# patriciogonzalezvivo/prisma

Measured on AMD Instinct MI355X. Metric: frames/sec (depth_anything ViT-L + flow_raft, 1080p), higher is better.
Workload: dtype split-f16

## Files before the change

include/prisma_bands.h:

```cpp
#ifndef PRISMA_BANDS_H
#define PRISMA_BANDS_H

#include <stddef.h>
#include <stdint.h>

#ifdef __cplusplus
extern "C" {
#endif

typedef struct pb_ctx pb_ctx;

typedef enum {
    PB_OK = 0,
    PB_ERR_ARG = -1,
    PB_ERR_DEVICE = -2,
    PB_ERR_MEMORY = -3,
    PB_ERR_STATE = -4
} pb_status;

typedef enum { PB_F32 = 0, PB_F16 = 1, PB_U8 = 2, PB_I32 = 3 } pb_dtype;

typedef struct {
    const char *name;
    int32_t dtype;
// ... 102 lines not shown
                           float *flow_out, uint8_t *rgb_out, float *maxdisp_out);
int pb_flow_infer_sequence_dev(pb_ctx *ctx, const uint8_t *frames, int F, int H, int W, float scale, int iters, int backward,
                               float *flow_out, uint8_t *rgb_out, float *maxdisp_out);
int pb_flow_infer_sequence_masks(pb_ctx *ctx, const uint8_t *frames, int F, int H, int W, float scale, int iters,
                                 float alpha1, float alpha2, float *flow_out, uint8_t *rgb_out, float *maxdisp_out,
                                 uint8_t *mask_out);
int pb_flow_infer_sequence_masks_dev(pb_ctx *ctx, const uint8_t *frames, int F, int H, int W, float scale, int iters,
                                     float alpha1, float alpha2, float *flow_out, uint8_t *rgb_out, float *maxdisp_out,
                                     uint8_t *mask_out);
int pb_flow_fwdbwd_mask(pb_ctx *ctx, const float *flows, int n, int sh, int sw, float alpha1, float alpha2,
                        uint8_t *mask_out);
int pb_flow_num_scales(pb_ctx *ctx);
int64_t pb_flow_get_stage(pb_ctx *ctx, const char *name, float *out, int64_t cap, int64_t shape_out[4]);
int pb_flow_set_inference_size(pb_ctx *ctx, int h, int w);
int pb_flow_set_matching(pb_ctx *ctx, int corr_radius, int prop_radius);
int pb_flow_set_alternate_corr(pb_ctx *ctx, int on);
int64_t pb_flow_arena_bytes(pb_ctx *ctx);

int pb_mask_infer_batch(pb_ctx *ctx, const uint8_t *frames, int n, int H, int W, float confidence,
                        const int32_t *keep_classes, int n_keep, uint8_t *mask_out);
int pb_mask_infer_batch_dev(pb_ctx *ctx, const uint8_t *frames, int n, int H, int W, float confidence,
                            const int32_t *keep_classes, int n_keep, uint8_t *mask_out);
int pb_mask_get_instances(pb_ctx *ctx, int frame, int cap, float *scores_out, int32_t *labels_out, uint8_t *masks_out,
                          int32_t *candidates_out);
int pb_mask_net_size(const pb_mask_cfg *cfg, int H, int W, int *nh, int *nw, int *Hp, int *Wp);
int pb_mask_set_sdf(pb_ctx *ctx, const uint8_t *tab_out, const uint8_t *tab_in, int n_tab);
int pb_mask_sdf_green(pb_ctx *ctx, uint8_t *masks, int n, int H, int W);
int pb_mask_sdf_green_dev(pb_ctx *ctx, uint8_t *masks, int n, int H, int W);
int64_t pb_mask_get_stage(pb_ctx *ctx, const char *name, float *out, int64_t cap, int64_t shape_out[4]);

int64_t pb_depth_get_stage(pb_ctx *ctx, const char *name, float *out, int64_t cap, int64_t shape_out[4]);

int pb_dev_alloc(pb_ctx *ctx, void **ptr, size_t bytes);
int pb_dev_free(pb_ctx *ctx, void *ptr);
int pb_memcpy_h2d(pb_ctx *ctx, void *dst, const void *src, size_t bytes);
int pb_memcpy_d2h(pb_ctx *ctx, void *dst, const void *src, size_t bytes);

typedef struct {
    const char *name;
    double ms;
    double flops;
    double exec_flops;
    double bytes;
    int32_t launches;
} pb_kernel_stat;
int pb_set_profiling(pb_ctx *ctx, int enabled);
int pb_set_option(pb_ctx *ctx, const char *key, int value);
int pb_get_kernel_stats(pb_ctx *ctx, pb_kernel_stat *out, int cap);

int pb_op_gemm(pb_ctx *ctx, const float *A, const float *W, const float *bias, float *C,
               int M, int N, int K, int act , int tile );
int pb_op_gemm_bench(pb_ctx *ctx, int M, int N, int K, int tile, int epi, int iters, double *ms_out);
int pb_op_corr_volume(pb_ctx *ctx, const float *A, int M, const float *W, int N, int ldo, int guard_rows, float *out);
int pb_op_attention_bench(pb_ctx *ctx, int B, int heads, int N, int variant, int iters, double *ms_out);
int pb_op_layernorm(pb_ctx *ctx, const float *x, const float *g, const float *b, float *y, int rows, int D);
int pb_op_attention(pb_ctx *ctx, const float *q, const float *k, const float *v, float *o,
                    int B, int heads, int N);
int pb_op_attention128(pb_ctx *ctx, const float *q, const float *k, const float *v, const int8_t *region, float *o, int B, int L);
int pb_op_attention128_split(pb_ctx *ctx, const float *q, const float *k, const float *v, const int8_t *region, int nreg, float *o,
                             int B, int L, int vcols, int kxor);
int pb_op_conv2d(pb_ctx *ctx, const float *x, const float *w, const float *bias, float *y,
                 int B, int Ci, int H, int W, int Co, int ksize, int stride, int pad, int relu_in, int relu_out);
int pb_op_conv2d_split(pb_ctx *ctx, const float *x, const float *w, const float *bias, const float *skip, int B, int H, int W, int Ci, int Ctot,
                       int ci_off, int Co, int kh, int kw, int stride, int layout, int sa, int tapin, int tile, int split_out, int act,
                       int pre_relu, int rows_out, void *out, int *info, char *kernel, int kernel_cap);
int pb_op_dense_split(pb_ctx *ctx, const float *A, const float *w, const float *bias, const float *skip, int M, int K, int N, int layout,
                      int sa, int tile, int split_out, int act, int rows_out, void *out, int *info, char *kernel, int kernel_cap);
int pb_op_gemm_resid(pb_ctx *ctx, const float *A, const float *w, const float *bias, const float *gamma, const float *X, int M, int N, int K, int ldr,
                     int layout, int tile, int guard_rows, float *out, int *info, char *kernel, int kernel_cap);
int pb_op_gemm_qkv(pb_ctx *ctx, const float *A, const float *w, const float *bias, int B, int ntp, int D, int layout, int tile, int guard_rows, void *q,
                   void *k, void *vt, int *info, char *kernel, int kernel_cap);
int pb_op_gemm_patch(pb_ctx *ctx, const float *A, const float *w, const float *bias, const float *pos, int B, int P, int ntp, int D, int layout,
                     int guard_rows, float *out, int *info, char *kernel, int kernel_cap);
int pb_op_raft_gru_zr(pb_ctx *ctx, const float *x, const float *w, const float *bias, const float *add1, const float *add2, float *h32, int n, int H, int W,
                      int gc, int kh, int kw, int layout, int tile, int guard_rows, void *zrb, void *rh, int *info, char *kernel, int kernel_cap);
int pb_op_raft_gru_q(pb_ctx *ctx, const float *x, const float *w, const float *bias, const float *add1, const float *add2, const float *z, float *h32, int n,
                     int H, int W, int gc, int kh, int kw, int layout, int tile, int guard_rows, void *out, int *info, char *kernel, int kernel_cap);
int pb_op_conv_pixshuf(pb_ctx *ctx, const float *x, const float *w, const float *bias, int B, int H, int W, int layout, int act, int guard_rows, void *out,
                       int *info, char *kernel, int kernel_cap);
int pb_op_gemm_fc1(pb_ctx *ctx, const float *A, const float *w, const float *bias, int M, int K, int N, int tile, int guard_rows, void *out, int *info,
                   char *kernel, int kernel_cap);
int pb_op_gemm_pixshuf(pb_ctx *ctx, const float *x, const float *wt, const float *bias, int B, int h, int w, int C, int s, int layout, int tile,
                       int guard_rows, void *out, int *info, char *kernel, int kernel_cap);
int pb_op_conv_head(pb_ctx *ctx, const float *x, const float *w, const float *bias, const float *w2, float b2, int B, int H, int W, int C, int layout,
                    int guard_rows, float *out, int *info, char *kernel, int kernel_cap);
int pb_op_raft_geometry(int h8, int w8, int *geo);
int pb_op_raft_lookup(pb_ctx *ctx, const float *fmap1, const float *fmap2, const float *flow, int n, int h8, int w8, int o8, int guard_rows,
                      void *out, float *levels);
int pb_op_raft_lookup_otf(pb_ctx *ctx, const float *fmap1, const float *fmap2, const float *flow, int n, int h8, int w8, int o8,
                          int guard_rows, void *out);
int pb_op_raft_convf1(pb_ctx *ctx, const float *flow, const float *w, const float *bias, int n, int h8, int w8, int passes, int o8,
                      int gemm_path, int guard_rows, void *out);
int pb_op_raft_flow_head2(pb_ctx *ctx, const float *x, const float *w, const float *bias, float *flow, int n, int H, int W, int split,
                          int guard_rows);
int pb_op_raft_upsample(pb_ctx *ctx, const float *flow, const float *mask, int n, int h8, int w8, int pad_l, int pad_t, int sh, int sw,
                        int guard, float *up, float *maxd);
int pb_op_raft_instnorm(pb_ctx *ctx, const float *a, const float *b, int B, int HW, int C, int layout, int stats_lo, int bmode, int inplace,
                        int guard_rows, float *stats, void *out);
int pb_op_raft_state(pb_ctx *ctx, const float *ctx_rows, const float *flow, int rows, int ld, int inp_off, int guard_rows, float *h32, void *hx,
                     void *hx2, float *flow0);
int pb_op_gm_tables(int h8, int w8, float *pos, int8_t *region);
int pb_op_gm_tables_n(int h, int w, int splits, float *pos, int8_t *region);
int pb_op_gm_tokens_warped(pb_ctx *ctx, const float *feat, const float *warped, const float *pos, int B, int dirs, int P, int guard_rows, float *X,
                           void *Xs);
int pb_op_gm_warp(pb_ctx *ctx, const float *flow8, const float *feat4, int B, int dirs, int h8, int w8, int guard_rows, float *flow_up,
                  float *warped);
// ... 82 lines not shown
```

prisma_amd/_lib.py:

```python
from __future__ import annotations

import ctypes as C
import os

_HERE = os.path.dirname(os.path.abspath(__file__))
LIB_PATH = os.environ.get("PRISMA_BANDS_LIB") or os.path.join(_HERE, "libprisma_bands.so")


class pb_tensor(C.Structure):
    _fields_ = [("name", C.c_char_p), ("dtype", C.c_int32), ("ndim", C.c_int32),
                ("shape", C.c_int64 * 6), ("data", C.c_void_p)]


class pb_depth_cfg(C.Structure):
    _fields_ = [("embed_dim", C.c_int32), ("depth", C.c_int32), ("heads", C.c_int32), ("features", C.c_int32),
                ("out_channels", C.c_int32 * 4), ("pos_grid", C.c_int32), ("max_batch", C.c_int32), ("metric", C.c_int32),
                ("precision", C.c_int32)]


class pb_flow_cfg(C.Structure):
    _fields_ = [("precision", C.c_int32)]


PREC_F16, PREC_SPLIT = 0, 1
# ... 39 lines not shown
    "pb_host_alloc": (C.c_int, [_P, C.POINTER(_P), C.c_size_t]),
    "pb_host_free": (C.c_int, [_P, _P]),
    "pb_comm_unique_id": (C.c_int, [_P]),
    "pb_comm_init": (C.c_int, [_P, _P, C.c_int, C.c_int]),
    "pb_gather_scalars": (C.c_int, [_P, _P, C.c_int, _P]),
    "pb_depth_encode_still": (C.c_int, [_P, _P, C.c_int, C.c_int, C.c_int, C.c_int, _P, _F, _F]),
    "pb_depth_point_cloud": (C.c_int, [_P, _P, _P, C.c_int, C.c_int, C.c_int, C.c_int] + [C.c_float] * 4 + [_P]),
    "pb_depth_point_cloud_dev": (C.c_int, [_P, _P, _P, C.c_int, C.c_int, C.c_int, C.c_int] + [C.c_float] * 4 + [_P]),
    "pb_rgbd_boxes": (C.c_int, [C.c_int, C.c_int, C.c_int, C.POINTER(C.c_int), C.POINTER(C.c_int)]),
    "pb_rgbd_depth": (C.c_int, [_P, _P, C.c_int, C.c_int, C.c_int, C.c_int, _P, _P]),
    "pb_rgbd_depth_dev": (C.c_int, [_P, _P, C.c_int, C.c_int, C.c_int, C.c_int, _P, _P]),
    "pb_i420_bytes": (C.c_int64, [C.c_int, C.c_int]),
    "pb_i420_to_rgb": (C.c_int, [_P, _P, C.c_int, C.c_int, C.c_int, _P]),
    "pb_i420_to_rgb_dev": (C.c_int, [_P, _P, C.c_int, C.c_int, C.c_int, _P]),
    "pb_rgb_to_i420": (C.c_int, [_P, _P, C.c_int, C.c_int, C.c_int, _P]),
    "pb_rgb_to_i420_dev": (C.c_int, [_P, _P, C.c_int, C.c_int, C.c_int, _P]),
    "pb_rgb_resize": (C.c_int, [_P, _P, C.c_int, C.c_int, C.c_int, C.c_int, C.c_int, _P, C.c_int]),
    "pb_rgb_resize_dev": (C.c_int, [_P, _P, C.c_int, C.c_int, C.c_int, C.c_int, C.c_int, _P, C.c_int]),
    "pb_depth_net_size": (C.c_int, [C.c_int, C.c_int, C.POINTER(C.c_int), C.POINTER(C.c_int)]),
    "pb_depth_get_stage": (C.c_int64, [_P, C.c_char_p, _P, C.c_int64, C.POINTER(C.c_int64)]),
    "pb_mask_infer_batch": (C.c_int, [_P, _P, C.c_int, C.c_int, C.c_int, C.c_float, _P, C.c_int, _P]),
    "pb_mask_infer_batch_dev": (C.c_int, [_P, _P, C.c_int, C.c_int, C.c_int, C.c_float, _P, C.c_int, _P]),
    "pb_mask_get_instances": (C.c_int, [_P, C.c_int, C.c_int, _P, _P, _P, _P]),
    "pb_mask_net_size": (C.c_int, [C.POINTER(pb_mask_cfg), C.c_int, C.c_int, C.POINTER(C.c_int), C.POINTER(C.c_int),
                                   C.POINTER(C.c_int), C.POINTER(C.c_int)]),
    "pb_mask_get_stage": (C.c_int64, [_P, C.c_char_p, _P, C.c_int64, C.POINTER(C.c_int64)]),
    "pb_flow_set_inference_size": (C.c_int, [_P, C.c_int, C.c_int]),
    "pb_flow_set_matching": (C.c_int, [_P, C.c_int, C.c_int]),
    "pb_flow_num_scales": (C.c_int, [_P]),
    "pb_flow_set_alternate_corr": (C.c_int, [_P, C.c_int]),
    "pb_flow_arena_bytes": (C.c_int64, [_P]),
    "pb_mask_set_sdf": (C.c_int, [_P, _P, _P, C.c_int]),
    "pb_mask_sdf_green": (C.c_int, [_P, _P, C.c_int, C.c_int, C.c_int]),
    "pb_mask_sdf_green_dev": (C.c_int, [_P, _P, C.c_int, C.c_int, C.c_int]),
    "pb_flow_out_size": (C.c_int, [C.c_int, C.c_int, C.c_float, C.POINTER(C.c_int), C.POINTER(C.c_int)]),
    "pb_flow_infer_sequence": (C.c_int, [_P, _P, C.c_int, C.c_int, C.c_int, C.c_float, C.c_int, C.c_int, _P, _P, _P]),
    "pb_flow_infer_sequence_dev": (C.c_int, [_P, _P, C.c_int, C.c_int, C.c_int, C.c_float, C.c_int, C.c_int, _P, _P, _P]),
    "pb_flow_infer_sequence_masks": (C.c_int, [_P, _P, C.c_int, C.c_int, C.c_int, C.c_float, C.c_int, C.c_float, C.c_float,
                                               _P, _P, _P, _P]),
    "pb_flow_infer_sequence_masks_dev": (C.c_int, [_P, _P, C.c_int, C.c_int, C.c_int, C.c_float, C.c_int, C.c_float,
                                                   C.c_float, _P, _P, _P, _P]),
    "pb_flow_fwdbwd_mask": (C.c_int, [_P, _P, C.c_int, C.c_int, C.c_int, C.c_float, C.c_float, _P]),
    "pb_flow_get_stage": (C.c_int64, [_P, C.c_char_p, _P, C.c_int64, C.POINTER(C.c_int64)]),
    "pb_dev_alloc": (C.c_int, [_P, C.POINTER(_P), C.c_size_t]),
    "pb_dev_free": (C.c_int, [_P, _P]),
    "pb_memcpy_h2d": (C.c_int, [_P, _P, _P, C.c_size_t]),
    "pb_memcpy_d2h": (C.c_int, [_P, _P, _P, C.c_size_t]),
    "pb_set_profiling": (C.c_int, [_P, C.c_int]),
    "pb_set_option": (C.c_int, [_P, C.c_char_p, C.c_int]),
    "pb_get_kernel_stats": (C.c_int, [_P, C.POINTER(pb_kernel_stat), C.c_int]),
    "pb_op_gemm": (C.c_int, [_P, _P, _P, _P, _P, C.c_int, C.c_int, C.c_int, C.c_int, C.c_int]),
    "pb_op_gemm_bench": (C.c_int, [_P, C.c_int, C.c_int, C.c_int, C.c_int, C.c_int, C.c_int, C.POINTER(C.c_double)]),
    "pb_op_corr_volume": (C.c_int, [_P, _P, C.c_int, _P, C.c_int, C.c_int, C.c_int, _P]),
    "pb_op_attention_bench": (C.c_int, [_P, C.c_int, C.c_int, C.c_int, C.c_int, C.c_int, C.POINTER(C.c_double)]),
    "pb_op_layernorm": (C.c_int, [_P, _P, _P, _P, _P, C.c_int, C.c_int]),
    "pb_op_attention": (C.c_int, [_P, _P, _P, _P, _P, C.c_int, C.c_int, C.c_int]),
    "pb_op_attention128": (C.c_int, [_P, _P, _P, _P, _P, _P, C.c_int, C.c_int]),
    "pb_op_attention128_split": (C.c_int, [_P, _P, _P, _P, _P, C.c_int, _P, C.c_int, C.c_int, C.c_int, C.c_int]),
    "pb_op_conv2d": (C.c_int, [_P, _P, _P, _P, _P] + [C.c_int] * 10),
    "pb_op_conv2d_split": (C.c_int, [_P, _P, _P, _P, _P] + [C.c_int] * 18 + [_P, _P, _P, C.c_int]),
    "pb_op_dense_split": (C.c_int, [_P, _P, _P, _P, _P] + [C.c_int] * 9 + [_P, _P, _P, C.c_int]),
    "pb_op_gemm_resid": (C.c_int, [_P, _P, _P, _P, _P, _P] + [C.c_int] * 7 + [_P, _P, _P, C.c_int]),
    "pb_op_gemm_qkv": (C.c_int, [_P, _P, _P, _P] + [C.c_int] * 6 + [_P, _P, _P, _P, _P, C.c_int]),
    "pb_op_gemm_patch": (C.c_int, [_P, _P, _P, _P, _P] + [C.c_int] * 6 + [_P, _P, _P, C.c_int]),
    "pb_op_raft_gru_zr": (C.c_int, [_P, _P, _P, _P, _P, _P, _P] + [C.c_int] * 9 + [_P, _P, _P, _P, C.c_int]),
    "pb_op_raft_gru_q": (C.c_int, [_P, _P, _P, _P, _P, _P, _P, _P] + [C.c_int] * 9 + [_P, _P, _P, C.c_int]),
    "pb_op_conv_pixshuf": (C.c_int, [_P, _P, _P, _P] + [C.c_int] * 6 + [_P, _P, _P, C.c_int]),
    "pb_op_gemm_fc1": (C.c_int, [_P, _P, _P, _P] + [C.c_int] * 5 + [_P, _P, _P, C.c_int]),
    "pb_op_gemm_pixshuf": (C.c_int, [_P, _P, _P, _P] + [C.c_int] * 8 + [_P, _P, _P, C.c_int]),
    "pb_op_conv_head": (C.c_int, [_P, _P, _P, _P, _P, C.c_float] + [C.c_int] * 6 + [_P, _P, _P, C.c_int]),
    "pb_op_raft_geometry": (C.c_int, [C.c_int, C.c_int, C.POINTER(C.c_int)]),
    "pb_op_raft_lookup": (C.c_int, [_P, _P, _P, _P] + [C.c_int] * 5 + [_P, _P]),
    "pb_op_raft_lookup_otf": (C.c_int, [_P, _P, _P, _P] + [C.c_int] * 5 + [_P]),
    "pb_op_raft_convf1": (C.c_int, [_P, _P, _P, _P] + [C.c_int] * 7 + [_P]),
    "pb_op_raft_flow_head2": (C.c_int, [_P, _P, _P, _P, _P] + [C.c_int] * 5),
    "pb_op_raft_upsample": (C.c_int, [_P, _P, _P] + [C.c_int] * 8 + [_P, _P]),
    "pb_op_raft_instnorm": (C.c_int, [_P, _P, _P] + [C.c_int] * 8 + [_P, _P]),
    "pb_op_raft_state": (C.c_int, [_P, _P, _P] + [C.c_int] * 4 + [_P, _P, _P, _P]),
    "pb_op_gm_tables": (C.c_int, [C.c_int, C.c_int, _P, _P]),
    "pb_op_gm_tables_n": (C.c_int, [C.c_int, C.c_int, C.c_int, _P, _P]),
    "pb_op_gm_tokens_warped": (C.c_int, [_P, _P, _P, _P] + [C.c_int] * 4 + [_P, _P]),
    "pb_op_gm_warp": (C.c_int, [_P, _P, _P] + [C.c_int] * 5 + [_P, _P]),
    "pb_op_gm_upsample": (C.c_int, [_P, _P, _P] + [C.c_int] * 9 + [_P, _P]),
    "pb_op_gm_pack_n": (C.c_int, [_P, _P] + [C.c_int] * 6 + [_P, _P, C.c_int, C.c_int, _P]),
    "pb_op_gm_ln_n": (C.c_int, [_P, _P, _P, _P, _P] + [C.c_int] * 9 + [_P]),
    "pb_op_gm_window_block_n": (C.c_int, [_P, _P, _P, _P, _P] + [C.c_int] * 8),
    "pb_op_gm_tokens": (C.c_int, [_P, _P, _P, C.c_int, C.c_int, C.c_int, _P, _P]),
    "pb_op_gm_split_rows": (C.c_int, [_P, _P] + [C.c_int] * 4 + [_P]),
    "pb_op_gm_grid_vt": (C.c_int, [_P] + [C.c_int] * 3 + [_P]),
    "pb_op_gm_pack": (C.c_int, [_P, _P] + [C.c_int] * 5 + [_P, _P, C.c_int, C.c_int, _P]),
    "pb_op_gm_ln": (C.c_int, [_P, _P, _P, _P, _P] + [C.c_int] * 8 + [_P]),
    "pb_op_gm_match_flow": (C.c_int, [_P, _P] + [C.c_int] * 4 + [_P, _P]),
    "pb_op_gm_upsampler_in": (C.c_int, [_P, _P, _P] + [C.c_int] * 5 + [_P, _P]),
    "pb_op_attention128_cfg": (C.c_int, [_P, _P, _P, _P, _P, C.c_int, _P] + [C.c_int] * 9 + [C.c_float]),
    "pb_op_gm_window_block": (C.c_int, [_P, _P, _P, _P, _P] + [C.c_int] * 6),
    "pb_op_gm_match": (C.c_int, [_P, _P] + [C.c_int] * 5 + [_P]),
    "pb_op_gm_propagate": (C.c_int, [_P, _P, _P, _P, _P] + [C.c_int] * 6 + [_P, _P, _P]),
    "pb_op_gm_local_match": (C.c_int, [_P, _P] + [C.c_int] * 6 + [_P]),
    "pb_op_gm_local_propagate": (C.c_int, [_P, _P, _P, _P] + [C.c_int] * 6 + [_P]),
    "pb_op_mask_prep": (C.c_int, [_P, _P] + [C.c_int] * 7 + [_P, _P, C.c_int, C.c_int, _P, _P]),
    "pb_op_mask_maxpool": (C.c_int, [_P, _P] + [C.c_int] * 6 + [_P]),
    "pb_op_mask_nearest_add": (C.c_int, [_P, _P, _P] + [C.c_int] * 8 + [_P]),
    "pb_op_mask_subsample2": (C.c_int, [_P, _P] + [C.c_int] * 6 + [_P]),
    "pb_op_mask_coord_concat": (C.c_int, [_P, _P] + [C.c_int] * 7 + [_P]),
    "pb_op_mask_bilinear": (C.c_int, [_P, _P, _P] + [C.c_int] * 10 + [_P]),
    "pb_op_mask_gn_relu": (C.c_int, [_P, _P, _P, _P] + [C.c_int] * 5 + [_P, _P]),
# ... 60 lines not shown
```

prisma_amd/csrc/abi.hip:

```cpp
#include <dlfcn.h>
#include <stdarg.h>
#include <stdlib.h>
#include <string.h>

#include <algorithm>

#include "abi_ctx.h"
#include "gmflow_engine.h"
#include "raft_engine.h"

static thread_local char g_err[1024] = "";

void pb_set_error(const char *fmt, ...) {
    va_list ap;
    va_start(ap, fmt);
    vsnprintf(g_err, sizeof(g_err), fmt, ap);
    va_end(ap);
}

static bool pb_is_pinned(const void *p, size_t bytes = 1) {
    if (!p) return false;
    for (const char *q : {(const char *)p, (const char *)p + (bytes ? bytes - 1 : 0)}) {
        hipPointerAttribute_t at;
        if (hipPointerGetAttributes(&at, q) != hipSuccess) { (void)hipGetLastError(); return false; }
// ... 594 lines not shown
int64_t pb_mask_get_stage(pb_ctx *c, const char *name, float *out, int64_t cap, int64_t shape_out[4]) {
    return band_stage(c, c ? c->mask : nullptr, "mask ", name, out, cap, shape_out);
}

int pb_flow_set_inference_size(pb_ctx *c, int h, int w) {
    PB_CHECK(c && c->flow, PB_ERR_STATE, "ctx has no flow band");
    GmflowEngine *g = dynamic_cast<GmflowEngine *>(c->flow);
    PB_CHECK(g, PB_ERR_STATE, "--inference_size is a flow_gmflow option");
    return g->set_inference_size(h, w);
}

int pb_flow_set_matching(pb_ctx *c, int corr_radius, int prop_radius) {
    PB_CHECK(c && c->flow, PB_ERR_STATE, "ctx has no flow band");
    GmflowEngine *g = dynamic_cast<GmflowEngine *>(c->flow);
    PB_CHECK(g, PB_ERR_STATE, "--corr_radius_list / --prop_radius_list are flow_gmflow options");
    return g->set_matching(corr_radius, prop_radius);
}

int pb_flow_num_scales(pb_ctx *c) {
    PB_CHECK(c && c->flow, PB_ERR_ARG, "ctx has no flow band");
    GmflowEngine *g = dynamic_cast<GmflowEngine *>(c->flow);
    PB_CHECK(g, PB_ERR_ARG, "num_scales is a flow_gmflow property");
    return g->num_scales();
}

int pb_flow_set_alternate_corr(pb_ctx *c, int on) {
    PB_CHECK(c && c->flow, PB_ERR_ARG, "ctx has no flow band");
    RaftEngine *e = dynamic_cast<RaftEngine *>(c->flow);
    PB_CHECK(e, PB_ERR_ARG, "--alternate_corr is a flow_raft option");
    e->set_alternate_corr(on);
    return 0;
}

int64_t pb_flow_arena_bytes(pb_ctx *c) {
    PB_CHECK(c && c->flow, PB_ERR_ARG, "ctx has no flow band");
    return c->flow->plan_bytes();
}

int64_t pb_flow_get_stage(pb_ctx *c, const char *name, float *out, int64_t cap, int64_t shape_out[4]) {
    return band_stage(c, c ? c->flow : nullptr, "flow ", name, out, cap, shape_out);
}

int pb_set_option(pb_ctx *c, const char *key, int value) {
    PB_CHECK(c && key, PB_ERR_ARG, "set_option: bad arguments");
    if (!strcmp(key, "gemm_tile")) (c->band ? c->band->dense_tile : c->gemm_tile) = value;
    else if (!strcmp(key, "conv_tile")) (c->band ? c->band->conv_tile : c->conv_tile) = value;
    else if (!strcmp(key, "host_chunk")) c->host_chunk = value;
    else if (!strcmp(key, "op_splitk")) c->op_splitk = value;
    else if (!strcmp(key, "frames_i420") || !strcmp(key, "rgb_out_i420") || !strcmp(key, "rgb_out_full")) {
        PB_CHECK(value == 0 || value == 1, PB_ERR_ARG, "option '%s' is 0 or 1, not %d", key, value);
        PB_CHECK(c->pending.empty(), PB_ERR_STATE, "option '%s': a submission of this ctx is still outstanding (pb_wait first)", key);
        (key[0] == 'f' ? c->frames_i420 : key[8] == 'i' ? c->rgb_out_i420 : c->rgb_out_full) = value;
    }
    else if (!strcmp(key, "tile_n96")) pb_gemm_set_n96(value);
    else PB_CHECK(false, PB_ERR_ARG, "unknown option '%s'", key);
    return 0;
}

int pb_get_kernel_stats(pb_ctx *c, pb_kernel_stat *out, int cap) {
    PB_CHECK(c && c->band && out, PB_ERR_STATE, "ctx has no band");
    return c->band->stats(out, cap);
}

int pb_dev_alloc(pb_ctx *c, void **ptr, size_t bytes) {
    PB_CHECK(c && ptr, PB_ERR_ARG, "dev_alloc: bad arguments");
    PB_HIP(hipSetDevice(c->device));
    hipError_t e = hipMalloc(ptr, bytes);
    PB_CHECK(e == hipSuccess, PB_ERR_MEMORY, "hipMalloc(%zu): %s", bytes, hipGetErrorString(e));
    return 0;
}
int pb_dev_free(pb_ctx *c, void *ptr) {
    PB_CHECK(c, PB_ERR_ARG, "null ctx");
    PB_HIP(hipSetDevice(c->device));
    PB_HIP(hipFree(ptr));
    return 0;
}
int pb_host_alloc(pb_ctx *c, void **ptr, size_t bytes) {
    PB_CHECK(c && ptr, PB_ERR_ARG, "host_alloc: bad arguments");
    *ptr = nullptr;
    PB_HIP(hipSetDevice(c->device));
    void *p = nullptr;
    hipError_t e = hipHostMalloc(&p, bytes ? bytes : 1, hipHostMallocDefault);
    if (e != hipSuccess) (void)hipGetLastError();
    PB_CHECK(e == hipSuccess && p, PB_ERR_MEMORY, "hipHostMalloc(%zu): %s", bytes, hipGetErrorString(e));
    std::lock_guard<std::mutex> lock(c->host_mu);
    c->host_blocks.push_back(p);
    *ptr = p;
    return 0;
}
int pb_host_free(pb_ctx *c, void *ptr) {
    PB_CHECK(c, PB_ERR_ARG, "null ctx");
    {
        std::lock_guard<std::mutex> lock(c->host_mu);
        auto it = std::find(c->host_blocks.begin(), c->host_blocks.end(), ptr);
        PB_CHECK(ptr && it != c->host_blocks.end(), PB_ERR_ARG, "host_free: %p is not a block pb_host_alloc gave this ctx", ptr);
        c->host_blocks.erase(it);
    }
    PB_HIP(hipSetDevice(c->device));
    PB_HIP(hipHostFree(ptr));
    return 0;
}
int pb_memcpy_h2d(pb_ctx *c, void *dst, const void *src, size_t bytes) {
    PB_CHECK(c, PB_ERR_ARG, "null ctx");
    PB_HIP(hipSetDevice(c->device));
    PB_HIP(hipMemcpy(dst, src, bytes, hipMemcpyHostToDevice));
    return 0;
// ... 176 lines not shown
```

prisma_amd/csrc/abi_ctx.h:

```cpp
#pragma once
#include <deque>
#include <mutex>
#include <vector>

#include "engine.h"
#include "mask_engine.h"
#include "flow_engine.h"
#include "resize.h"
#include "yuv.h"

void pb_cubic_taps(int src, int dst, int *idx, float *wt);

#define PB_TRY(expr) do { int _r = (expr); if (_r) return _r; } while (0)

struct ChunkPipe {
    static constexpr int kLanes = 5;
    hipStream_t s_in = nullptr, s_out = nullptr;
    hipEvent_t ev_h2d[2] = {}, ev_comp[2] = {}, ev_d2h[2] = {};
    struct Lane { void *h[2] = {}, *d[2] = {}; size_t cap = 0; } lane[kLanes];
    unsigned seq = 0;
    int grow(int k, size_t need, bool host) {
        Lane &l = lane[k];
        if (need <= l.cap && (!host || l.h[0] || !need)) return 0;
        const size_t want = need > l.cap ? need : l.cap;
// ... 48 lines not shown
        }
        if (bytes > cap_d) {
            if (d_in) PB_HIP(hipFree(d_in));
            if (d_out) PB_HIP(hipFree(d_out));
            d_in = d_out = nullptr; cap_d = 0;
            PB_HIP(hipMalloc(&d_in, bytes));
            PB_HIP(hipMalloc(&d_out, bytes));
            cap_d = bytes;
        }
        if (host_in && bytes > cap_hi) {
            if (h_in) PB_HIP(hipHostFree(h_in));
            h_in = nullptr; cap_hi = 0;
            PB_HIP(hipHostMalloc(&h_in, bytes, hipHostMallocDefault));
            cap_hi = bytes;
        }
        if (host_out && bytes > cap_ho) {
            if (h_out) PB_HIP(hipHostFree(h_out));
            h_out = nullptr; cap_ho = 0;
            PB_HIP(hipHostMalloc(&h_out, bytes, hipHostMallocDefault));
            cap_ho = bytes;
        }
        while ((int)ev_in.size() < chunks) {
            hipEvent_t a, b;
            PB_HIP(hipEventCreateWithFlags(&a, hipEventDisableTiming));
            PB_HIP(hipEventCreateWithFlags(&b, hipEventDisableTiming));
            ev_in.push_back(a); ev_done.push_back(b);
        }
        return 0;
    }
    void release() {
        if (s_in) { hipStreamSynchronize(s_in); hipStreamSynchronize(s_out); }
        if (d_in) hipFree(d_in);
        if (d_out) hipFree(d_out);
        if (h_in) hipHostFree(h_in);
        if (h_out) hipHostFree(h_out);
        for (auto e : ev_in) hipEventDestroy(e);
        for (auto e : ev_done) hipEventDestroy(e);
        if (s_in) { hipStreamDestroy(s_in); hipStreamDestroy(s_out); }
    }
};

struct pb_ctx {
    int device = 0;
    DepthEngine *depth = nullptr;
    FlowEngine *flow = nullptr;
    MaskEngine *mask = nullptr;
    EngineBase *band = nullptr;
    hipStream_t stream = nullptr;
    f16 *zero = nullptr;
    bool own_stream = false;
    int gemm_tile = TILE_AUTO, conv_tile = TILE_AUTO;
    int op_splitk = 0;
    int host_chunk = 0;
    ChunkPipe pipe;
    MaskPipe mpipe;
    std::deque<hipEvent_t> pending;
    std::vector<void *> host_blocks;
    std::mutex host_mu;
    void *comm = nullptr;
    int comm_rank = 0, comm_world = 0;
    float *comm_buf = nullptr;
    size_t comm_cap = 0;
    hipStream_t still_stream = nullptr;
    char *still_buf = nullptr;
    size_t still_cap = 0;
    std::mutex still_mu;
    int frames_i420 = 0, rgb_out_i420 = 0, rgb_out_full = 0;
    void *yuv[2] = {};
    size_t yuv_cap[2] = {};
    int yuv_grow(int k, size_t need) {
        if (need <= yuv_cap[k]) return 0;
        PB_HIP(hipStreamSynchronize(stream));
        if (yuv[k]) PB_HIP(hipFree(yuv[k]));
        yuv[k] = nullptr; yuv_cap[k] = 0;
        PB_HIP(hipMalloc(&yuv[k], need));
        yuv_cap[k] = need;
        return 0;
    }
    unsigned *pcl_mm = nullptr;
    int pcl_mm_cap = 0;
};
```

prisma_amd/csrc/abi_ops.hip:

```cpp
#include <string.h>

#include <algorithm>
#include <vector>

#include "abi_ctx.h"
#include "gmflow_engine.h"
#include "mask_kernels.h"
#include "zoe_kernels.h"

namespace {
enum { SL_F16 = 0, SL_SPLIT16 = 1, SL_MX3 = 2, SL_MX2 = 3 };

class SplitOpEngine : public EngineBase {
  public:
    explicit SplitOpEngine(int device) : EngineBase(device) {}
    int setup(const pb_tensor *t, int n, int layout, int tapin) {
        PB_TRY(begin_load(t, n));
        split_w_ = layout != SL_F16; mx_ = layout >= SL_MX3; pack_mx2_ = layout == SL_MX2; pack_tapin_ = tapin;
        return 0;
    }
    int pack_layer(bool is_conv, int sa, int N, int K, PackedW &w) {
        if (is_conv) return pack_conv("l", true, nullptr, nullptr, w, sa);
        const pb_tensor *tw = find("l.weight"), *tb = find("l.bias");
        PB_CHECK(tw && tb, PB_ERR_ARG, "split op: no weights");
        return pack((const float *)tw->data, N, K, (int)round_up(K, 64), w, (const float *)tb->data, 1, sa);
    }
    void build_map(const float *x, int64_t P, int C, int Cp, int layout, int sa, int64_t ld, std::vector<f16> &h) const {
        for (int64_t p = 0; p < P; ++p) {
            f16 *row = h.data() + p * ld;
            unsigned char *r8 = (unsigned char *)(row + Cp);
            for (int c = 0; c < C; ++c) {
                const float v = x[p * C + c];
                const f16 hi = (f16)v;
                row[c] = hi;
                if (layout == SL_SPLIT16 && sa) row[Cp + c] = (f16)(v - (float)hi);
                if (layout == SL_MX3) {
                    r8[c] = pb_f32_to_e4m3(ldexpf((float)hi, kLo8Pa));
                    r8[Cp + c] = pb_f32_to_e4m3(ldexpf(v - (float)hi, kLo8Pa + 12));
                }
                if (layout == SL_MX2) r8[c] = pb_f32_to_e4m3(ldexpf((float)hi, kMx2Pa));
            }
        }
    }
    void build_skip(const float *s, int M, int N, int C, int lo_off, bool lo8, int64_t ldo, std::vector<f16> &h) const {
        for (int m = 0; m < M; ++m) {
            f16 *row = h.data() + (int64_t)m * ldo;
            unsigned char *r8 = (unsigned char *)(row + C);
            for (int n = 0; n < N; ++n) {
                const float v = s[(int64_t)m * N + n];
                const f16 hi = (f16)v;
                row[n] = hi;
                if (lo_off && lo8) {
                    r8[n] = pb_f32_to_e4m3(ldexpf((float)hi, kLo8Pa));
                    r8[C + n] = pb_f32_to_e4m3(ldexpf(v - (float)hi, kLo8Pa + 12));
                } else if (lo_off) {
                    row[C + n] = (f16)(v - (float)hi);
                }
            }
// ... 46 lines not shown
        PB_HIP(hipDeviceSynchronize());
        pb_gemm_set_last_kernel("");
        const f16 *in = dx.as<f16>() + (m2 ? ci_off : 0);
        int r;
        if (is_conv) {
            conv_tile = tile;
            r = conv(in, Cp, m2 ? (int)ld : 0, B, H, W, kh, kw, stride, w, dout.as<f16>(), (int)ldo, act, pre_relu, dskip.as<f16>(), nullptr, lo_off,
                     m2 ? Ctot - ci_off / 2 : 0);
        } else {
            dense_tile = tile;
            PB_CHECK(!pre_relu, PB_ERR_ARG, "split op: dense() has no pre_relu");
            r = dense(in, (int)ld, M, w, dout.as<f16>(), (int)ldo, act, dskip.as<f16>(), 0, -1, lo_off);
        }
        sk_ws_ = nullptr; sk_cap_ = 0;
        if (r) return r;
        PB_HIP(hipStreamSynchronize(stream));
        PB_HIP(hipMemcpy(out, dout.p, (size_t)rows_out * ldo * 2, hipMemcpyDeviceToHost));
        if (info) {
            const int v[13] = {w.mx_pw, m2 ? kMx2Pa : kLo8Pa, w.mx3, w.mx2, w.sa, w.sw, w.tapin, w.K, w.wcw != nullptr, w.Cseg, (int)ldo, lo8, kLo8Pa};
            memcpy(info, v, sizeof(v));
        }
        if (kname && kcap > 0) snprintf(kname, kcap, "%s", pb_gemm_last_kernel());
        return 0;
    }
};

class RaftOpEngine : public SplitOpEngine {
  public:
    explicit RaftOpEngine(int device) : SplitOpEngine(device) {}
    static int up(DevMem &d, const void *src, size_t bytes) {
        PB_TRY(d.alloc(bytes));
        PB_HIP(hipMemcpy(d.p, src, bytes, hipMemcpyHostToDevice));
        return 0;
    }
    static int preset(DevMem &d, size_t bytes) {
        PB_TRY(d.alloc(bytes));
        PB_HIP(hipMemset(d.p, 0xFF, bytes));
        PB_HIP(hipDeviceSynchronize());
        return 0;
    }
    int to_f16(DevMem &d, const float *x, int64_t rows, int C, size_t min_bytes = 0) {
        std::vector<f16> h((size_t)rows * C);
        build_map(x, rows, C, C, SL_F16, 0, C, h);
        PB_TRY(d.alloc(std::max(h.size() * 2, min_bytes)));
        PB_HIP(hipMemcpy(d.p, h.data(), h.size() * 2, hipMemcpyHostToDevice));
        return 0;
    }
    int finish(void *out, const DevMem &d, size_t bytes) {
        PB_HIP(hipStreamSynchronize(stream));
        PB_HIP(hipMemcpy(out, d.p, bytes, hipMemcpyDeviceToHost));
        return 0;
    }

    int lookup(const float *fmap1, const float *fmap2, const float *flow, int n, int h8, int w8, int o8, int guard_rows, void *out, float *levels) {
        PB_CHECK(h8 >= 16 && w8 >= 16, PB_ERR_ARG, "op_raft_lookup: a %d x %d grid is too small (the 4-level pyramid needs >= 16 x 16)", h8, w8);
        CorrGeo g;
        corr_pyramid_geometry(h8, w8, g);
        const int P = h8 * w8;
        const int64_t rows = (int64_t)n * P;
        const size_t slack = 1 << 20;
        const int ldo = o8 ? 576 : 384;
        DevMem f1, f2, dflow, dout, fpool[4], ftile[4], pyr[4];
        PB_TRY(to_f16(f1, fmap1, rows, 256, (size_t)round_up(rows, 256) * 256 * 2 + slack));
        PB_TRY(to_f16(f2, fmap2, rows, 256, (size_t)round_up(rows, 256) * 256 * 2 + slack));
        PB_TRY(up(dflow, flow, (size_t)rows * 8));
        PB_TRY(preset(dout, (size_t)(rows + guard_rows) * ldo * 2));
        const f16 *lv[4];
        for (int l = 0; l < 4; ++l) {
            PB_TRY(pyr[l].alloc((size_t)rows * g.ld[l] * 2 + slack));
            if (l) PB_TRY(fpool[l].alloc((size_t)round_up((int64_t)n * g.h[l] * g.w[l], 256) * 256 * 2 + slack));
            PB_TRY(ftile[l].alloc((size_t)(n * (int64_t)g.ld[l] + 256) * 256 * 2 + slack));
            lv[l] = pyr[l].as<f16>();
        }
        for (int l = 0; l < 4; ++l) {
            if (l > 0) PB_TRY(launch_avgpool2_nhwc(stream, l == 1 ? f2.as<f16>() : fpool[l - 1].as<f16>(), fpool[l].as<f16>(), n, g.h[l - 1], g.w[l - 1], 256));
            PB_TRY(launch_corr_tile(stream, l == 0 ? f2.as<f16>() : fpool[l].as<f16>(), ftile[l].as<f16>(), n, g.h[l], g.w[l], g.wp[l], g.ld[l]));
        }
        for (int i = 0; i < n; ++i)
            for (int l = 0; l < 4; ++l)
                PB_TRY(launch_corr_volume(stream, f1.as<f16>() + (int64_t)i * P * 256, P, ftile[l].as<f16>() + (int64_t)i * g.ld[l] * 256, g.ld[l], g.ld[l],
                                          pyr[l].as<f16>() + (int64_t)i * P * g.ld[l], g.ld[l]));
        PB_TRY(launch_corr_lookup(stream, lv, g.h, g.w, g.wp, g.hp, g.ld, dflow.as<float>(), P, w8, dout.as<f16>(), rows, ldo, o8 ? 768 : 0,
                                  (float)(1 << kMx2Pa)));
        PB_TRY(finish(out, dout, (size_t)(rows + guard_rows) * ldo * 2));
        if (levels) {
            float *dst = levels;
            for (int l = 0; l < 4; ++l) {
                std::vector<f16> h((size_t)rows * g.ld[l]);
                PB_HIP(hipMemcpy(h.data(), pyr[l].p, h.size() * 2, hipMemcpyDeviceToHost));
                const int wt = g.wp[l] >> 3;
                for (int64_t r = 0; r < rows; ++r)
                    for (int y = 0; y < g.h[l]; ++y)
                        for (int x = 0; x < g.w[l]; ++x)
                            *dst++ = (float)h[(size_t)r * g.ld[l] + ((y >> 3) * wt + (x >> 3)) * 64 + (y & 7) * 8 + (x & 7)];
            }
        }
        return 0;
    }

    int lookup_otf(const float *fmap1, const float *fmap2, const float *flow, int n, int h8, int w8, int o8, int guard_rows, void *out) {
        PB_CHECK(h8 >= 16 && w8 >= 16, PB_ERR_ARG, "op_raft_lookup_otf: a %d x %d grid is too small (the 4-level pyramid needs >= 16 x 16)", h8, w8);
        CorrGeo g;
        corr_pyramid_geometry(h8, w8, g);
        const int P = h8 * w8;
        const int64_t rows = (int64_t)n * P;
        const size_t slack = 1 << 20;
        const int ldo = o8 ? 576 : 384;
        DevMem f1, f2, dflow, dout, fpool[4];
        PB_TRY(to_f16(f1, fmap1, rows, 256, (size_t)round_up(rows, 256) * 256 * 2 + slack));
        PB_TRY(to_f16(f2, fmap2, rows, 256, (size_t)round_up(rows, 256) * 256 * 2 + slack));
        PB_TRY(up(dflow, flow, (size_t)rows * 8));
        PB_TRY(preset(dout, (size_t)(rows + guard_rows) * ldo * 2));
        for (int l = 1; l < 4; ++l) {
            PB_TRY(fpool[l].alloc((size_t)round_up((int64_t)n * g.h[l] * g.w[l], 256) * 256 * 2 + slack));
            PB_TRY(launch_avgpool2_nhwc(stream, l == 1 ? f2.as<f16>() : fpool[l - 1].as<f16>(), fpool[l].as<f16>(), n, g.h[l - 1], g.w[l - 1], 256));
        }
        const f16 *const tg[4] = {f2.as<f16>(), fpool[1].as<f16>(), fpool[2].as<f16>(), fpool[3].as<f16>()};
        PB_TRY(launch_corr_lookup_otf(stream, f1.as<f16>(), tg, g.h, g.w, dflow.as<float>(), P, w8, dout.as<f16>(), rows, ldo, o8 ? 768 : 0,
                                      (float)(1 << kMx2Pa), 0));
        return finish(out, dout, (size_t)(rows + guard_rows) * ldo * 2);
    }

    int convf1(const float *flow, const float *wt, const float *bias, int n, int h8, int w8, int passes, int o8, int gemm, int guard_rows, void *out) {
        const int P = h8 * w8, ldo = o8 ? 192 : 128;
        const int64_t rows = (int64_t)n * P, rows_buf = round_up(rows + guard_rows, 256);
        DevMem dflow, dout, dw, db, fa;
        PB_TRY(up(dflow, flow, (size_t)rows * 8));
        PB_TRY(preset(dout, (size_t)rows_buf * ldo * 2));
        if (!gemm) {
            std::vector<f16> hw((size_t)convf1_packed_halfs(passes));
            convf1_pack(wt, passes, hw.data());
            PB_TRY(up(dw, hw.data(), hw.size() * 2));
            PB_TRY(up(db, bias, 128 * 4));
            PB_TRY(launch_convf1(stream, dflow.as<float>(), dw.as<f16>(), db.as<float>(), dout.as<f16>(), rows, P, h8, w8, ldo, o8 ? 256 : 0,
                                 (float)(1 << kMx2Pa), passes));
        } else {
            PB_CHECK(passes == 2 || !o8, PB_ERR_ARG, "op_raft_convf1: the GEMM path reads fp8 copies only in the split mode");
            split_w_ = passes == 2; mx_ = o8; pack_mx2_ = o8; pack_tapin_ = 0;
            std::vector<float> g((size_t)128 * 98);
            for (int o = 0; o < 128; ++o)
                for (int c = 0; c < 2; ++c)
                    for (int tp = 0; tp < 49; ++tp) g[(size_t)o * 98 + tp * 2 + c] = wt[((size_t)o * 2 + c) * 49 + tp];
            PackedW w;
            PB_TRY(pack(g.data(), 128, 98, 128, w, bias));
            PB_TRY(fa.alloc((size_t)round_up(rows, 256) * ldo * 2));
            PB_TRY(launch_im2col7_flow(stream, dflow.as<float>(), n, h8, w8, fa.as<f16>(), 128, ldo, o8));
            PB_TRY(dense(fa.as<f16>(), ldo, rows, w, dout.as<f16>(), ldo, ACT_RELU, nullptr, o8 ? 256 : 0, 0));
// ... 968 lines not shown
extern "C" {

int pb_op_gemm(pb_ctx *c, const float *A, const float *W, const float *bias, float *C, int M, int N, int K, int act,
               int tile) {
    PB_CHECK(c && A && W && C && M > 0 && N > 0 && K > 0 && N % 8 == 0, PB_ERR_ARG, "op_gemm: bad arguments");
    PB_HIP(hipSetDevice(c->device));
    const int Kp = (int)round_up(K, 64), Np = (int)round_up(N, 256);
    const int64_t Mp = round_up(M, 256);
    DevMem a32, w32, b32, a16, w16, c16, c32;
    PB_TRY(a32.alloc((size_t)M * K * 4)); PB_TRY(w32.alloc((size_t)N * K * 4));
    PB_TRY(a16.alloc((size_t)Mp * Kp * 2)); PB_TRY(w16.alloc((size_t)Np * Kp * 2));
    PB_TRY(c16.alloc((size_t)Mp * N * 2)); PB_TRY(c32.alloc((size_t)M * N * 4));
    PB_HIP(hipMemcpy(a32.p, A, (size_t)M * K * 4, hipMemcpyHostToDevice));
    PB_HIP(hipMemcpy(w32.p, W, (size_t)N * K * 4, hipMemcpyHostToDevice));
    if (bias) {
        PB_TRY(b32.alloc((size_t)N * 4));
        PB_HIP(hipMemcpy(b32.p, bias, (size_t)N * 4, hipMemcpyHostToDevice));
    }
    PB_TRY(launch_f32_to_f16(c->stream, a32.as<float>(), a16.as<f16>(), M, K, Kp));
    PB_TRY(launch_f32_to_f16(c->stream, w32.as<float>(), w16.as<f16>(), N, K, Kp));
    GemmArgs g;
    g.A = a16.as<f16>(); g.lda = Kp; g.W = w16.as<f16>(); g.K = Kp; g.M = M; g.N = N;
    g.bias = b32.as<float>(); g.out = c16.as<f16>(); g.ldo = N; g.act = act; g.zero = c->zero;
    DevMem skw;
    PB_TRY(lend_splitk(c, skw, g));
    PB_TRY(launch_gemm(c->stream, A_DENSE, EPI_STD, tile, g));
    PB_TRY(launch_f16_to_f32(c->stream, c16.as<f16>(), c32.as<float>(), M, N, N));
    PB_HIP(hipStreamSynchronize(c->stream));
    PB_HIP(hipMemcpy(C, c32.p, (size_t)M * N * 4, hipMemcpyDeviceToHost));
    return 0;
}

int pb_op_corr_volume(pb_ctx *c, const float *A, int M, const float *W, int N, int ldo, int guard_rows, float *out) {
    PB_CHECK(c && A && W && out && M > 0 && N > 0 && N % 8 == 0 && ldo >= N && guard_rows >= 0, PB_ERR_ARG, "op_corr_volume: bad arguments");
    PB_HIP(hipSetDevice(c->device));
    const int64_t rows = (int64_t)M + guard_rows, Np = round_up(N, 64);
    DevMem a32, w32, a16, w16, o16, o32;
    PB_TRY(a32.alloc((size_t)M * 256 * 4)); PB_TRY(w32.alloc((size_t)N * 256 * 4));
    PB_TRY(a16.alloc((size_t)M * 256 * 2)); PB_TRY(w16.alloc((size_t)Np * 256 * 2));
    PB_TRY(o16.alloc((size_t)rows * ldo * 2)); PB_TRY(o32.alloc((size_t)rows * ldo * 4));
    PB_HIP(hipMemcpy(a32.p, A, (size_t)M * 256 * 4, hipMemcpyHostToDevice));
    PB_HIP(hipMemcpy(w32.p, W, (size_t)N * 256 * 4, hipMemcpyHostToDevice));
    PB_HIP(hipMemsetAsync(w16.p, 0, (size_t)Np * 256 * 2, c->stream));
    PB_HIP(hipMemsetAsync(o16.p, 0x7e, (size_t)rows * ldo * 2, c->stream));
    PB_TRY(launch_f32_to_f16(c->stream, a32.as<float>(), a16.as<f16>(), M, 256, 256));
    PB_TRY(launch_f32_to_f16(c->stream, w32.as<float>(), w16.as<f16>(), N, 256, 256));
    PB_TRY(launch_corr_volume(c->stream, a16.as<f16>(), M, w16.as<f16>(), N, (int)Np, o16.as<f16>(), ldo));
    PB_TRY(launch_f16_to_f32(c->stream, o16.as<f16>(), o32.as<float>(), rows, ldo, ldo));
    PB_HIP(hipStreamSynchronize(c->stream));
    PB_HIP(hipMemcpy(out, o32.p, (size_t)rows * ldo * 4, hipMemcpyDeviceToHost));
    return 0;
}

int pb_op_gemm_bench(pb_ctx *c, int M, int N, int K, int tile, int epi, int iters, double *ms_out) {
    PB_CHECK(c && M > 0 && N > 0 && K > 0 && K % 64 == 0 && N % 8 == 0 && iters > 0 && ms_out, PB_ERR_ARG, "gemm_bench: bad arguments");
    PB_HIP(hipSetDevice(c->device));
    DevMem a, w, o, r, b;
    const int64_t Mp = round_up(M, 256), Np = round_up(N, 256);
    PB_TRY(a.alloc((size_t)Mp * K * 2)); PB_TRY(w.alloc((size_t)Np * K * 2)); PB_TRY(o.alloc((size_t)Mp * N * 2));
    PB_TRY(r.alloc((size_t)Mp * N * 4)); PB_TRY(b.alloc((size_t)Np * 4));
    PB_TRY(launch_fill_random_f16(c->stream, a.as<f16>(), (int64_t)M * K, 1u, 1.f));
    PB_TRY(launch_fill_random_f16(c->stream, w.as<f16>(), (int64_t)N * K, 2u, 0.05f));
    GemmArgs g;
    g.A = a.as<f16>(); g.lda = K; g.W = w.as<f16>(); g.K = K; g.M = M; g.N = N; g.zero = c->zero; g.bias = b.as<float>();
    int e = EPI_STD, amode = A_DENSE;
    if (epi == 2) { e = EPI_RESID; g.resid = r.as<float>(); g.ldr = N; g.gamma = b.as<float>(); }
    else { g.out = o.as<f16>(); g.ldo = N; g.act = epi == 1 ? ACT_GELU : ACT_NONE; }
    if (epi >= 10) {
        const int taps = epi == 12 ? 5 : 9;
        PB_CHECK(M % 18360 == 0 && K % (taps * 64) == 0, PB_ERR_ARG, "gemm_bench: conv modes need M = B * 102 * 180 and K = taps * C");
        amode = A_CONV;
        g.cH = g.cOH = 102; g.cW = g.cOW = 180; g.cC = K / taps; g.cStride = 1;
        if (epi == 12) { g.cKW = 5; g.cPad = 0; g.cPadX = 2; g.cKH = 1; }
        else { g.cKW = 3; g.cPad = 1; g.cKH = 3; g.cTapInner = epi == 11; }
    }
    const BenchEnv benv = bench_env();
    g.ablate = benv.gemm_abl;
    for (int i = 0; i < 2; ++i) PB_TRY(launch_gemm(c->stream, amode, e, tile, g));
    if (!benv.gemm_dbg.empty()) {
        const int nblk = (int)((Mp / 256) * (Np / 256));
        DevMem d;
        PB_TRY(d.alloc((size_t)nblk * 64));
        g.dbg = d.as<long long>();
        PB_TRY(launch_gemm(c->stream, amode, e, tile, g));
        PB_HIP(hipStreamSynchronize(c->stream));
        std::vector<long long> h((size_t)nblk * 8);
        PB_HIP(hipMemcpy(h.data(), d.p, h.size() * 8, hipMemcpyDeviceToHost));
        if (FILE *f = fopen(benv.gemm_dbg.c_str(), "wb")) { fwrite(h.data(), 8, h.size(), f); fclose(f); }
        g.dbg = nullptr;
    }
    return time_launches(c->stream, iters, ms_out, [&] { return launch_gemm(c->stream, amode, e, tile, g); });
}

int pb_op_attention_bench(pb_ctx *c, int B, int heads, int N, int variant, int iters, double *ms_out) {
    PB_CHECK(c && B > 0 && heads > 0 && N > 0 && iters > 0 && ms_out, PB_ERR_ARG, "attention_bench: bad arguments");
    PB_HIP(hipSetDevice(c->device));
    const int ntp = (int)round_up(N, 16), D = heads * 64;
    const size_t n = (size_t)B * heads * ntp * 64;
    DevMem dq, dk, dv, dout;
    PB_TRY(dq.alloc(n * 2 + 32768)); PB_TRY(dk.alloc(n * 2 + 32768)); PB_TRY(dv.alloc(n * 2 + 32768));
    PB_TRY(dout.alloc((size_t)B * ntp * D * 2));
    PB_TRY(launch_fill_random_f16(c->stream, dq.as<f16>(), (int64_t)n, 11u, 3.f * PB_QSCALE));
    PB_TRY(launch_fill_random_f16(c->stream, dk.as<f16>(), (int64_t)n, 12u, 3.f));
    PB_TRY(launch_fill_random_f16(c->stream, dv.as<f16>(), (int64_t)n, 13u, 1.f));
    auto launch = [&] { return launch_attention(c->stream, dq.as<f16>(), dk.as<f16>(), dv.as<f16>(), dout.as<f16>(), B, heads, ntp, N, D, variant); };
    for (int i = 0; i < 2; ++i) PB_TRY(launch());
// ... 256 lines not shown
    PB_CHECK(c && x && w && bias && w2 && out && B > 0 && H > 0 && W > 0 && C > 0 && guard_rows >= 0, PB_ERR_ARG, "op_conv_head: bad arguments");
    EPI_OP_ENGINE(e);
    return e.head(c, x, w, bias, w2, b2, B, H, W, C, layout, guard_rows, out, info, kernel, kernel_cap);
}
int pb_op_conv_pixshuf(pb_ctx *c, const float *x, const float *w, const float *bias, int B, int H, int W, int layout, int act, int guard_rows, void *out,
                       int *info, char *kernel, int kernel_cap) {
    PB_CHECK(c && x && w && bias && out && B > 0 && H > 0 && W > 0 && (act == ACT_NONE || act == ACT_RELU) && guard_rows >= 0, PB_ERR_ARG,
             "op_conv_pixshuf: bad arguments");
    EPI_OP_ENGINE(e);
    return e.pixshuf_conv(c, x, w, bias, B, H, W, layout, act, guard_rows, out, info, kernel, kernel_cap);
}
int pb_op_raft_gru_zr(pb_ctx *c, const float *x, const float *w, const float *bias, const float *add1, const float *add2, float *h32, int n, int H, int W,
                      int gc, int kh, int kw, int layout, int tile, int guard_rows, void *zrb, void *rh, int *info, char *kernel, int kernel_cap) {
    PB_CHECK(c && x && w && bias && h32 && zrb && rh && n > 0 && H > 0 && W > 0 && (gc == 256 || gc == 384) && kh >= 1 && kw >= 1 && guard_rows >= 0,
             PB_ERR_ARG, "op_raft_gru_zr: bad arguments");
    PB_HIP(hipSetDevice(c->device));
    EpiOpEngine e(c->device);
    return e.gru(c, 0, x, w, bias, add1, add2, nullptr, h32, n, H, W, gc, kh, kw, layout, tile, guard_rows, zrb, rh, info, kernel, kernel_cap);
}
int pb_op_raft_gru_q(pb_ctx *c, const float *x, const float *w, const float *bias, const float *add1, const float *add2, const float *z, float *h32, int n,
                     int H, int W, int gc, int kh, int kw, int layout, int tile, int guard_rows, void *out, int *info, char *kernel, int kernel_cap) {
    PB_CHECK(c && x && w && bias && z && h32 && out && n > 0 && H > 0 && W > 0 && (gc == 256 || gc == 384) && kh >= 1 && kw >= 1 && guard_rows >= 0,
             PB_ERR_ARG, "op_raft_gru_q: bad arguments");
    PB_HIP(hipSetDevice(c->device));
    EpiOpEngine e(c->device);
    return e.gru(c, 1, x, w, bias, add1, add2, z, h32, n, H, W, gc, kh, kw, layout, tile, guard_rows, out, nullptr, info, kernel, kernel_cap);
}
int pb_op_gemm_fc1(pb_ctx *c, const float *A, const float *w, const float *bias, int M, int K, int N, int tile, int guard_rows, void *out, int *info,
                   char *kernel, int kernel_cap) {
    PB_CHECK(c && A && w && bias && out && M > 0 && K > 0 && K % 64 == 0 && N > 0 && N % 64 == 0 && guard_rows >= 0, PB_ERR_ARG, "op_gemm_fc1: bad arguments");
    EPI_OP_ENGINE(e);
    return e.fc1(c, A, w, bias, M, K, N, tile, guard_rows, out, info, kernel, kernel_cap);
}
int pb_op_gemm_pixshuf(pb_ctx *c, const float *x, const float *wt, const float *bias, int B, int h, int w, int C, int s, int layout, int tile,
                       int guard_rows, void *out, int *info, char *kernel, int kernel_cap) {
    PB_CHECK(c && x && wt && bias && out && B > 0 && h > 0 && w > 0 && C > 0 && C % 8 == 0 && s >= 1 && s <= 4 && guard_rows >= 0, PB_ERR_ARG,
             "op_gemm_pixshuf: bad arguments");
    EPI_OP_ENGINE(e);
    return e.pixshuf(c, x, wt, bias, B, h, w, C, s, layout, tile, guard_rows, out, info, kernel, kernel_cap);
}

int pb_op_raft_geometry(int h8, int w8, int *geo) {
    PB_CHECK(geo && h8 >= 1 && w8 >= 1, PB_ERR_ARG, "op_raft_geometry: bad arguments");
    CorrGeo g;
    corr_pyramid_geometry(h8, w8, g);
    for (int l = 0; l < 4; ++l) { geo[l * 5] = g.h[l]; geo[l * 5 + 1] = g.w[l]; geo[l * 5 + 2] = g.wp[l]; geo[l * 5 + 3] = g.hp[l]; geo[l * 5 + 4] = g.ld[l]; }
    return 0;
}
#define RAFT_OP_ENGINE(e) PB_HIP(hipSetDevice(c->device)); RaftOpEngine e(c->device); PB_TRY(e.setup(nullptr, 0, SL_F16, 0))
int pb_op_raft_lookup(pb_ctx *c, const float *fmap1, const float *fmap2, const float *flow, int n, int h8, int w8, int o8, int guard_rows, void *out,
                      float *levels) {
    PB_CHECK(c && fmap1 && fmap2 && flow && out && n > 0 && guard_rows >= 0, PB_ERR_ARG, "op_raft_lookup: bad arguments");
    RAFT_OP_ENGINE(e);
    return e.lookup(fmap1, fmap2, flow, n, h8, w8, o8, guard_rows, out, levels);
}
int pb_op_raft_lookup_otf(pb_ctx *c, const float *fmap1, const float *fmap2, const float *flow, int n, int h8, int w8, int o8, int guard_rows, void *out) {
    PB_CHECK(c && fmap1 && fmap2 && flow && out && n > 0 && guard_rows >= 0, PB_ERR_ARG, "op_raft_lookup_otf: bad arguments");
    RAFT_OP_ENGINE(e);
    return e.lookup_otf(fmap1, fmap2, flow, n, h8, w8, o8, guard_rows, out);
}
int pb_op_raft_convf1(pb_ctx *c, const float *flow, const float *w, const float *bias, int n, int h8, int w8, int passes, int o8, int gemm_path,
                      int guard_rows, void *out) {
    PB_CHECK(c && flow && w && bias && out && n > 0 && h8 > 0 && w8 > 0 && (passes == 1 || passes == 2) && guard_rows >= 0, PB_ERR_ARG,
             "op_raft_convf1: bad arguments");
    RAFT_OP_ENGINE(e);
    return e.convf1(flow, w, bias, n, h8, w8, passes, o8, gemm_path, guard_rows, out);
}
int pb_op_raft_flow_head2(pb_ctx *c, const float *x, const float *w, const float *bias, float *flow, int n, int H, int W, int split, int guard_rows) {
    PB_CHECK(c && x && w && bias && flow && n > 0 && H > 0 && W > 0 && guard_rows >= 0, PB_ERR_ARG, "op_raft_flow_head2: bad arguments");
    PB_HIP(hipSetDevice(c->device));
    LayerTensors l(w, bias, 2, 256, 3, 3);
    RaftOpEngine e(c->device);
    PB_TRY(e.setup(l.t, 2, SL_F16, 0));
    return e.flow_head2(x, flow, n, H, W, split, guard_rows);
}
int pb_op_raft_upsample(pb_ctx *c, const float *flow, const float *mask, int n, int h8, int w8, int pad_l, int pad_t, int sh, int sw, int guard,
                        float *up, float *maxd) {
    PB_CHECK(c && flow && mask && up && maxd && n > 0 && h8 > 0 && w8 > 0 && sh > 0 && sw > 0 && pad_l >= 0 && pad_t >= 0 && guard >= 0 &&
             pad_t + sh <= 8 * h8 && pad_l + sw <= 8 * w8, PB_ERR_ARG, "op_raft_upsample: bad arguments");
    RAFT_OP_ENGINE(e);
    return e.upsample(flow, mask, n, h8, w8, pad_l, pad_t, sh, sw, guard, up, maxd);
}
int pb_op_raft_instnorm(pb_ctx *c, const float *a, const float *b, int B, int HW, int C, int layout, int stats_lo, int bmode, int inplace,
                        int guard_rows, float *stats, void *out) {
    PB_CHECK(c && a && stats && out && B > 0 && HW > 0 && C > 0 && layout >= 0 && layout <= 2 && bmode >= 0 && bmode <= 2 && (b || !bmode) &&
             guard_rows >= 0, PB_ERR_ARG, "op_raft_instnorm: bad arguments");
    RAFT_OP_ENGINE(e);
    return e.instnorm(a, b, B, HW, C, layout, stats_lo, bmode, inplace, guard_rows, stats, out);
}
int pb_op_raft_state(pb_ctx *c, const float *ctx_rows, const float *flow, int rows, int ld, int inp_off, int guard_rows, float *h32, void *hx,
                     void *hx2, float *flow0) {
    PB_CHECK(c && ctx_rows && flow && h32 && hx && hx2 && flow0 && rows > 0 && (ld == 384 || ld == 576) && (inp_off == 128 || inp_off == 256) &&
             guard_rows >= 0, PB_ERR_ARG, "op_raft_state: bad arguments");
    RAFT_OP_ENGINE(e);
    return e.state(ctx_rows, flow, rows, ld, inp_off, guard_rows, h32, hx, hx2, flow0);
}

int pb_op_gm_tables(int h8, int w8, float *pos, int8_t *region) {
    PB_CHECK(pos && region && h8 >= 4 && w8 >= 4 && h8 % 2 == 0 && w8 % 2 == 0, PB_ERR_ARG, "op_gm_tables: bad arguments");
    std::vector<float> p;
    std::vector<int8_t> r;
    sine_positions(h8, w8, p);
    shift_regions(h8, w8, r);
    memcpy(pos, p.data(), p.size() * 4);
    memcpy(region, r.data(), r.size());
    return 0;
}
// ... 338 lines not shown
```

prisma_amd/csrc/raft_engine.h:

```cpp
#pragma once
#include "flow_engine.h"

class RaftEngine : public FlowEngine {
  public:
    explicit RaftEngine(int device, const CreateEnv &env = create_env()) : FlowEngine(device, env) {}
    int load(const pb_tensor *w, int n) override;
    int infer(const uint8_t *frames, int F, int H, int W, float scale, int iters, int backward, float *flow_out, uint8_t *rgb_out,
              float *maxdisp, uint8_t *mask_out = nullptr, float alpha1 = 0.05f, float alpha2 = 0.5f) override;
    void set_alternate_corr(int on) { alt_corr_ = on ? 1 : 0; }
    int chunk_pairs(int wanted, int H, int W, float scale, int dirs) const override;

  private:
    int prepare(int F, int H, int W, float scale, int dirs);
    Enc fnet_, cnet_;
    PackedW convc1_, convc2_, convf1_, convf2_, convm_, zr_[2], q_[2], fh1_, fh2_, mk0_, mk2_;
    f16 *f1w_ = nullptr;
    int f1_passes_ = 1;
    bool f1_direct_ = true;
    PackedW zr_in_[2], q_in_[2];
    int hoist_ = 0;
    f16 *gz_[2] = {}, *gq_[2] = {};

    int alt_corr_ = 0;
    int lh_[4] = {0, 0, 0, 0}, lw_[4] = {0, 0, 0, 0};
    f16 *fmap_ = nullptr, *ctx_ = nullptr;
    f16 *pyr_[4] = {};
    f16 *ftile_[4] = {};
    int lwp_[4] = {}, lhp_[4] = {};
    f16 *fpool_[4] = {};
    int pld_[4] = {};
    float *h32_ = nullptr, *flow_ = nullptr;
    f16 *hx_ = nullptr, *hx2_ = nullptr, *corr_ = nullptr, *c1_ = nullptr, *corflo_ = nullptr, *fa_ = nullptr, *f1_ = nullptr,
        *zrb_ = nullptr, *fh_ = nullptr, *m0_ = nullptr;
    int upd8_ = 0;
};
```

prisma_amd/csrc/raft_engine.hip:

```cpp
#include "raft_engine.h"
#include "flow_chunk.h"

#include <math.h>
#include <string.h>

#include <algorithm>

int RaftEngine::chunk_pairs(int wanted, int H, int W, float scale, int dirs) const {
    if (!hoist_) return wanted;
    return flow_chunk_pairs(wanted, dirs, flow_geometry(H, W, scale, 8).P, upd8_ ? 576 : 384);
}

int RaftEngine::load(const pb_tensor *w, int n) {
    int r0 = begin_load(w, n);
    if (r0) return r0;
    int r;
    pack_tapin_ = env.tapin == 2;
    for (int e = 0; e < 2; ++e) {
        const std::string en = e == 0 ? "fnet" : "cnet";
        Enc &E = e == 0 ? fnet_ : cnet_;
        if ((r = pack_encoder(en, e == 1, true, E))) return r;
        if ((r = pack_conv(en + ".conv2", true, nullptr, nullptr, E.out, 1))) return r;
    }
    const std::string u = "update_block.";
    pack_mx2_ = mx_ && env.mx_upd;
    upd8_ = pack_mx2_;
    const int tapin_all = pack_tapin_;
    pack_tapin_ = env.tapin != 0;
    if ((r = pack_conv(u + "encoder.convc1", true, nullptr, nullptr, convc1_))) return r;
    if ((r = pack_conv(u + "encoder.convc2", true, nullptr, nullptr, convc2_))) return r;
    if ((r = pack_conv(u + "encoder.convf2", true, nullptr, nullptr, convf2_))) return r;
    if ((r = pack_conv(u + "encoder.conv", true, nullptr, nullptr, convm_))) return r;
    convm_.N = 128; convm_.Nreal = 126;
    {
        auto iw = tmap_.find(u + "encoder.convf1.weight"), ib = tmap_.find(u + "encoder.convf1.bias");
        PB_CHECK(iw != tmap_.end() && ib != tmap_.end(), PB_ERR_ARG, "missing convf1");
        const float *wt = (const float *)iw->second->data;
        std::vector<float> g((size_t)128 * 98);
        for (int o = 0; o < 128; ++o)
            for (int c = 0; c < 2; ++c)
                for (int tp = 0; tp < 49; ++tp) g[(size_t)o * 98 + tp * 2 + c] = wt[((size_t)o * 2 + c) * 49 + tp];
        if ((r = pack(g.data(), 128, 98, 128, convf1_, (const float *)ib->second->data))) return r;
        {
            f1_direct_ = env.convf1_direct;
            f1_passes_ = split_w_ ? 2 : 1;
            std::vector<f16> hw((size_t)convf1_packed_halfs(f1_passes_));
            convf1_pack(wt, f1_passes_, hw.data());
            void *pw = nullptr;
            PB_HIP(hipMalloc(&pw, hw.size() * 2));
            owned_.push_back(pw);
            PB_HIP(hipMemcpy(pw, hw.data(), hw.size() * 2, hipMemcpyHostToDevice));
            f1w_ = (f16 *)pw;
        }
    }
// ... 15 lines not shown
                    for (int tp = 0; tp < 5; ++tp) g[(size_t)(row0 + o) * 5 * width + tp * width + dst + c] = wt[((size_t)o * 384 + c0 + c) * 5 + tp];
        };
        std::vector<float> bb(256);
        for (int o = 0; o < 128; ++o) { bb[o] = ((const float *)bz->data)[o]; bb[128 + o] = ((const float *)br->data)[o]; }
        if (!hoist_) {
            const int K = 5 * 384;
            std::vector<float> g((size_t)256 * K, 0.f);
            fill(g, 0, 384, 0, wz, 0, 384);
            fill(g, 128, 384, 0, wr, 0, 384);
            if ((r = pack(g.data(), 256, K, K, zr_[half], bb.data(), 5))) return r;
            if ((r = pack_conv(u + "gru.convq" + sfx, true, nullptr, nullptr, q_[half]))) return r;
            continue;
        }
        {
            std::vector<float> g((size_t)256 * 5 * 256, 0.f), gi((size_t)256 * 5 * 128, 0.f);
            fill(g, 0, 256, 0, wz, 0, 128);   fill(g, 0, 256, 128, wz, 256, 128);
            fill(g, 128, 256, 0, wr, 0, 128); fill(g, 128, 256, 128, wr, 256, 128);
            fill(gi, 0, 128, 0, wz, 128, 128);
            fill(gi, 128, 128, 0, wr, 128, 128);
            if ((r = pack(g.data(), 256, 5 * 256, 5 * 256, zr_[half], bb.data(), 5))) return r;
            pack_mx2_ = 0;
            r = pack(gi.data(), 256, 5 * 128, 5 * 128, zr_in_[half], nullptr, 5);
            pack_mx2_ = upd8_;
            if (r) return r;
        }
        {
            std::vector<float> g((size_t)128 * 5 * 256, 0.f), gi((size_t)128 * 5 * 128, 0.f);
            fill(g, 0, 256, 0, wq, 0, 128); fill(g, 0, 256, 128, wq, 256, 128);
            fill(gi, 0, 128, 0, wq, 128, 128);
            if ((r = pack(g.data(), 128, 5 * 256, 5 * 256, q_[half], (const float *)bq->data, 5))) return r;
            pack_mx2_ = 0;
            r = pack(gi.data(), 128, 5 * 128, 5 * 128, q_in_[half], nullptr, 5);
            pack_mx2_ = upd8_;
            if (r) return r;
        }
    }
    if ((r = pack_conv(u + "flow_head.conv1", true, nullptr, nullptr, fh1_))) return r;
    pack_mx2_ = 0;
    const int tapin_upd = pack_tapin_;
    pack_tapin_ = 0;
    if ((r = pack_conv(u + "flow_head.conv2", true, nullptr, nullptr, fh2_))) return r;
    fh2_.N = 8;
    pack_mx2_ = upd8_;
    pack_tapin_ = tapin_upd;
    if ((r = pack_conv(u + "mask.0", true, nullptr, nullptr, mk0_))) return r;
    pack_mx2_ = 0;
    pack_tapin_ = tapin_all;
    if ((r = pack_conv(u + "mask.2", true, nullptr, nullptr, mk2_))) return r;
    tmap_.clear();
    PB_HIP(hipDeviceSynchronize());
    return 0;
}

int RaftEngine::prepare(int F, int H, int W, float scale, int dirs) {
    if (plan_.covers(F, H, W, scale, dirs, alt_corr_)) return 0;
    PB_HIP(hipStreamSynchronize(stream));
    plan_.clear();
    geometry(H, W, scale, 8);
    PB_CHECK(h8_ >= 16 && w8_ >= 16, PB_ERR_ARG, "flow_raft: %dx%d is too small (the 4-level pyramid needs >= 128 px)", sh_, sw_);
    {
        CorrGeo g;
        corr_pyramid_geometry(h8_, w8_, g);
        for (int l = 0; l < 4; ++l) { lh_[l] = g.h[l]; lw_[l] = g.w[l]; lwp_[l] = g.wp[l]; lhp_[l] = g.hp[l]; pld_[l] = g.ld[l]; }
    }
    const int64_t ND = (int64_t)(F - 1) * dirs;
    const size_t slack = 1 << 20;
    int r = plan_arena("flow", [&]() -> int {
        carve_encoder(F);
        fmap_ = (f16 *)carve((size_t)round_up((int64_t)F * P_, 256) * 256 * 2 + slack);
        ctx_ = (f16 *)carve((size_t)round_up((int64_t)F * P_, 256) * 256 * 2);
        for (int l = 0; l < 4; ++l) {
            pyr_[l] = alt_corr_ ? nullptr : (f16 *)carve((size_t)ND * P_ * pld_[l] * 2 + slack);
            fpool_[l] = l == 0 ? nullptr : (f16 *)carve((size_t)round_up((int64_t)F * lh_[l] * lw_[l], 256) * 256 * 2 + slack);
            ftile_[l] = alt_corr_ ? nullptr : (f16 *)carve((size_t)(F * (int64_t)pld_[l] + 256) * 256 * 2 + slack);
        }
        const int64_t rows = round_up(ND * P_, 256);
        h32_ = (float *)carve((size_t)rows * 128 * 4); flow_ = (float *)carve((size_t)rows * 2 * 4);
        mask_ = (float *)carve((size_t)rows * 576 * 4);
        const int Lq = upd8_ ? 576 : 384;
        const size_t u8 = upd8_ ? 3 : 2;
        hx_ = (f16 *)carve((size_t)rows * 384 * u8); hx2_ = (f16 *)carve((size_t)rows * 384 * u8);
        corr_ = (f16 *)carve((size_t)rows * 384 * u8); c1_ = (f16 *)carve((size_t)rows * 256 * u8);
        corflo_ = (f16 *)carve((size_t)rows * 256 * u8); fa_ = (f16 *)carve((size_t)rows * 128 * u8);
        f1_ = (f16 *)carve((size_t)rows * 128 * u8); zrb_ = (f16 *)carve((size_t)rows * 256 * 2);
        fh_ = (f16 *)carve((size_t)rows * 256 * 2);
        for (int half = 0; half < 2; ++half) {
            gz_[half] = hoist_ ? (f16 *)carve((size_t)rows * 256 * 2 * 2) : nullptr;
            gq_[half] = hoist_ ? (f16 *)carve((size_t)rows * Lq * 2 * 2) : nullptr;
        }
        m0_ = (f16 *)carve((size_t)rows * 256 * 2);
        up_ = (float *)carve((size_t)ND * sh_ * sw_ * 2 * 4);
        maxd_ = (unsigned *)carve((size_t)ND * 4);
        return 0;
    });
    if (r || (r = upload_resize_tables(H, W, scale))) return r;
    plan_.set(F, H, W, scale, dirs, alt_corr_);
    return 0;
}

int RaftEngine::infer(const uint8_t *frames, int F, int H, int W, float scale, int iters, int backward, float *flow_out,
                      uint8_t *rgb_out, float *maxdisp, uint8_t *mask_out, float alpha1, float alpha2) {
    PB_CHECK(frames && F >= 2 && H > 0 && W > 0 && iters >= 1 && scale > 0.f, PB_ERR_ARG, "flow infer: bad arguments");
    PB_CHECK(!mask_out || backward, PB_ERR_ARG, "consistency masks need both directions (backward = 1)");
    PB_HIP(hipSetDevice(device));
    const int dirs = backward ? 2 : 1;
    int r = prepare(F, H, W, scale, dirs);
    if (r) return r;
    timer.reset();
    stages_.clear();
    const int ND = (F - 1) * dirs;
    const int64_t rows = (int64_t)ND * P_;

    const int Lhx = upd8_ ? 576 : 384, L256 = upd8_ ? 384 : 256, L128 = upd8_ ? 192 : 128;
    const float s8 = (float)(1 << kMx2Pa);
    const int es = split_w_ ? 2 : 1;
    if ((r = prep_frames(frames, F, H, W, scale, split_w_ && mx_ ? kLo8Pa : -1))) return r;

    for (int e = 0; e < 2; ++e) {
        const Enc &E = e == 0 ? fnet_ : cnet_;
        const f16 *x = nullptr;
        const int Fe = e == 1 && dirs == 1 ? F - 1 : F;
        if ((r = run_encoder(E, e == 0, Fe, &x))) return r;
        if ((r = dense(x, es * 128, (int64_t)Fe * P_, E.out, e == 0 ? fmap_ : ctx_, 256, ACT_NONE))) return r;
    }
    stages_["fmap"] = Stage::f16_nhwc(fmap_, F, 256, h8_, w8_, 256);

    for (int l = 0; l < 4; ++l) {
        r = timed(F_ELT, 0, 0, [&] {
            int rc = l > 0 ? launch_avgpool2_nhwc(stream, l == 1 ? fmap_ : fpool_[l - 1], fpool_[l], F, lh_[l - 1], lw_[l - 1], 256) : 0;
            if (!rc && !alt_corr_) rc = launch_corr_tile(stream, l == 0 ? fmap_ : fpool_[l], ftile_[l], F, lh_[l], lw_[l], lwp_[l], pld_[l]);
            return rc;
        });
        if (r) return r;
    }
    for (int i = 0; i < F - 1; ++i)
        for (int d = 0; d < dirs; ++d) {
            const int n = i * dirs + d;
            for (int l = 0; l < 4 && !alt_corr_; ++l) {
                GemmArgs a;
                a.A = fmap_ + (int64_t)(i + d) * P_ * 256; a.lda = 256; a.M = P_;
                a.W = ftile_[l] + (int64_t)(i + 1 - d) * pld_[l] * 256;
                a.K = 256; a.N = pld_[l];
                a.out = pyr_[l] + (int64_t)n * P_ * pld_[l]; a.ldo = pld_[l]; a.zero = zero_;
                const double flops = 2.0 * P_ * (double)lh_[l] * lw_[l] * 256, bytes = 2.0 * ((double)P_ * 256 + (double)pld_[l] * 256 + (double)P_ * pld_[l]);
                if (!launch_env().volume)
                    r = timed_gemm(F_GEMM, flops, bytes, [&] { return launch_gemm(stream, A_DENSE, EPI_STD, TILE_AUTO, a); });
                else
                    r = timed(F_GEMM, flops, bytes, [&] { return launch_corr_volume(stream, a.A, a.M, a.W, a.N, a.N, a.out, a.ldo); }, "corr_volume_kernel");
                if (r) return r;
            }
            r = timed(F_ELT, 0, 0, [&] {
                return launch_init_state(stream, ctx_ + (int64_t)(i + d) * P_ * 256, h32_ + (int64_t)n * P_ * 128, hx_ + (int64_t)n * P_ * Lhx,
                                         hx2_ + (int64_t)n * P_ * Lhx, flow_ + (int64_t)n * P_ * 2, P_, Lhx, upd8_ ? 768 : 0, s8, hoist_ ? 256 : 128);
            });
            if (r) return r;
        }

    if (debug && (r = snapshot("net0", h32_, (size_t)ND * P_ * 128 * 4, Stage::f32_rows(nullptr, ND, P_, 128)))) return r;

    const int mot = hoist_ ? 128 : 256;
    if (hoist_) {
        PB_CHECK(rows * Lhx < (1LL << 31), PB_ERR_ARG, "flow_raft: %lld update-block rows exceed the 32-bit plane offset of the hoisted GRU share", (long long)rows);
        const int mx_saved = mx_;
        mx_ = 0;
        for (int half = 0; half < 2; ++half) {
            const int kh = half == 0 ? 1 : 5, kw = half == 0 ? 5 : 1;
            if ((r = conv(hx_ + 256, 128, Lhx, ND, h8_, w8_, kh, kw, 1, zr_in_[half], gz_[half], 256, ACT_NONE, 0, nullptr, nullptr, (int)(rows * 256)))) break;
            if ((r = conv(hx_ + 256, 128, Lhx, ND, h8_, w8_, kh, kw, 1, q_in_[half], gq_[half], Lhx, ACT_NONE, 0, nullptr, nullptr, (int)(rows * Lhx)))) break;
        }
        mx_ = mx_saved;
        if (r) return r;
    }

    for (int it = 0; it < iters; ++it) {
        if (alt_corr_) {
            const f16 *const tg[4] = {fmap_, fpool_[1], fpool_[2], fpool_[3]};
            r = timed(F_GEMM, 2.0 * rows * 4.0 * 100.0 * 256.0, 0, [&] {
                return launch_corr_lookup_otf(stream, fmap_, tg, lh_, lw_, flow_, P_, w8_, corr_, rows, Lhx, upd8_ ? 768 : 0, s8, dirs);
            }, "corr_lookup_otf_kernel");
        } else {
            r = timed(F_ELT, 0, 0, [&] { return launch_corr_lookup(stream, pyr_, lh_, lw_, lwp_, lhp_, pld_, flow_, P_, w8_, corr_, rows, Lhx, upd8_ ? 768 : 0, s8); });
        }
        if (r) return r;
        if (debug && it == 0 && (r = snapshot("corr0", corr_, (size_t)ND * P_ * Lhx * 2, Stage::f16_nhwc(nullptr, ND, 324, h8_, w8_, Lhx)))) return r;
        if ((r = conv(corr_, 384, Lhx, ND, h8_, w8_, 1, 1, 1, convc1_, c1_, L256, ACT_RELU, 0, nullptr, nullptr, 0, 0, upd8_ ? 512 : 0))) return r;
        if ((r = conv(c1_, 256, L256, ND, h8_, w8_, 3, 3, 1, convc2_, corflo_, L256, ACT_RELU, 0, nullptr, nullptr, 0, 0, upd8_ ? 512 : 0))) return r;
        if (f1_direct_) {
            r = timed(F_CONV, 2.0 * rows * 128.0 * 98.0, 8.0 * rows + 256.0 * rows, [&] {
                return launch_convf1(stream, flow_, f1w_, convf1_.bias, f1_, rows, P_, h8_, w8_, L128, upd8_ ? 256 : 0, (float)(1 << kMx2Pa), f1_passes_);
            }, "convf1_kernel", (double)f1_passes_);
            if (r) return r;
        } else {
            r = timed(F_ELT, 0, 0, [&] { return launch_im2col7_flow(stream, flow_, ND, h8_, w8_, fa_, 128, L128, upd8_); });
            if (r) return r;
            if ((r = dense(fa_, L128, rows, convf1_, f1_, L128, ACT_RELU, nullptr, upd8_ ? 256 : 0, 0))) return r;
        }
        if ((r = conv(f1_, 128, L128, ND, h8_, w8_, 3, 3, 1, convf2_, corflo_ + 192, L256, ACT_RELU, 0, nullptr, nullptr, 0, 0, upd8_ ? 512 - 192 : 0))) return r;
        ConvFuse dup; dup.out2 = hx2_ + mot;
        if ((r = conv(corflo_, 256, L256, ND, h8_, w8_, 3, 3, 1, convm_, hx_ + mot, Lhx, ACT_RELU, 0, nullptr, &dup, 0, 0, upd8_ ? 768 - mot : 0))) return r;
        r = timed(F_ELT, 0, 0, [&] { return launch_put_flow(stream, flow_, hx_, hx2_, rows, Lhx, upd8_ ? 768 : 0, s8, mot + 126); });
        if (r) return r;
        for (int half = 0; half < 2; ++half) {
            const int kh = half == 0 ? 1 : 5, kw = half == 0 ? 5 : 1;
            const int gc = hoist_ ? 256 : 384;
            ConvFuse fz; fz.gru_h = h32_; fz.gru_rh = hx2_; fz.gru_ld = Lhx; fz.add2 = hoist_ ? gz_[half] + rows * 256 : nullptr;
            const int a8 = upd8_ && hoist_ ? 384 : 0;
            if ((r = conv(hx_, gc, Lhx, ND, h8_, w8_, kh, kw, 1, zr_[half], zrb_, 256, ACT_GRU_ZR, 0, hoist_ ? gz_[half] : nullptr, &fz, 0, a8, upd8_ ? 768 : 0))) return r;
            ConvFuse fq; fq.gru_h = h32_; fq.gru_z = zrb_; fq.add2 = hoist_ ? gq_[half] + rows * Lhx : nullptr;
            if ((r = conv(hx2_, gc, Lhx, ND, h8_, w8_, kh, kw, 1, q_[half], hx_, Lhx, ACT_GRU_Q, 0, hoist_ ? gq_[half] : nullptr, &fq, 0, a8, upd8_ ? 768 : 0))) return r;
        }
        if ((r = conv(hx_, 128, Lhx, ND, h8_, w8_, 3, 3, 1, fh1_, fh_, 256, ACT_RELU, 0, nullptr, nullptr, 0, upd8_ ? 384 : 0))) return r;
        r = timed(F_CONV, 2.0 * rows * 2.0 * fh2_.Kreal, 0, [&] { return launch_flow_head2(stream, fh_, fh2_.w, fh2_.bias, flow_, ND, h8_, w8_, fh2_.sw); },
                  fh2_.sw ? "flow_head2_kernel<true>" : "flow_head2_kernel<false>");
        if (r) return r;
        if (debug && it == 0 && (r = snapshot("flow_it0", flow_, (size_t)ND * P_ * 2 * 4, Stage::f32_rows(nullptr, ND, P_, 2)))) return r;
    }
    stages_["flow_lo"] = Stage::f32_rows(flow_, ND, P_, 2);

    if ((r = conv(hx_, 128, Lhx, ND, h8_, w8_, 3, 3, 1, mk0_, m0_, 256, ACT_RELU, 0, nullptr, nullptr, 0, upd8_ ? 384 : 0))) return r;
    {
        GemmArgs a;
        a.A = m0_; a.lda = 256; a.N = 576; a.M = (int)rows;
        set_weights(a, mk2_, false);
        a.out32 = mask_; a.ldo = 576; a.scale = 0.25f;
        r = timed_gemm(F_GEMM, 2.0 * rows * 576.0 * 256, 0, [&] { return launch_gemm(stream, A_DENSE, EPI_F32, TILE_AUTO, a); }, 1.0 + mk2_.sw);
        if (r) return r;
    }
    return flow_tail(flow_, ND, F - 1, h8_, w8_, 8, flow_out, rgb_out, maxdisp, mask_out, alpha1, alpha2);
}
```

prisma_amd/csrc/raft_kernels.h:

```cpp
#pragma once
#include "common.h"

int launch_raft_prep(hipStream_t s, const uint8_t *frames, int F, int H, int W, int sh, int sw, int Hp, int Wp, int pad_l,
                     int pad_t, int resize, const int *xi, const int *xc, const int *yi, const int *yc, f16 *out,
                     uint8_t *scaled_out, int s2d = 0, int lo_off = 0, int lo8_pa = -1, int norm_mode = 0,
                     int isz = 0);
int launch_im2col7_flow(hipStream_t s, const float *x, int B, int H, int W, f16 *out, int Kp, int ld = 0, int o8 = 0);
int in_stats_chunks(int HW);
int launch_in_stats(hipStream_t s, const f16 *x, int B, int HW, int C, int ldc, float *part, float *stats, int lo_off = 0, int lo8_pa = -1);
int launch_in_apply(hipStream_t s, const f16 *a, const float *sa, const f16 *b, const float *sb, f16 *out, int B, int HW,
                    int C, int ldc, int lo_off = 0, int lo8_pa = -1);
int launch_init_state(hipStream_t s, const f16 *c, float *h32, f16 *hx, f16 *hx2, float *flow, int64_t rows, int ld = 384, int o8_off = 0,
                      float o8_scale = 16.f, int inp_off = 128);
int launch_avgpool2_nhwc(hipStream_t s, const f16 *x, f16 *y, int n, int H, int W, int C);
int launch_corr_tile(hipStream_t s, const f16 *x, f16 *y, int F, int h, int w, int wp, int npad);
int launch_corr_volume(hipStream_t s, const f16 *A, int M, const f16 *W, int N, int w_rows, f16 *out, int64_t ldo);
struct CorrGeo { int h[4], w[4], wp[4], hp[4], ld[4]; };
void corr_pyramid_geometry(int h8, int w8, CorrGeo &g);
int launch_corr_lookup(hipStream_t s, const f16 *const lv[4], const int h[4], const int w[4], const int wp[4], const int hp[4], const int ld[4],
                       const float *flow, int P, int w8, f16 *out, int64_t rows, int ldo = 384, int o8_off = 0, float o8_scale = 16.f);
int launch_corr_lookup_otf(hipStream_t s, const f16 *fmap_src, const f16 *const fmap_tgt[4], const int h[4], const int w[4], const float *flow, int P,
                           int w8, f16 *out, int64_t rows, int ldo = 384, int o8_off = 0, float o8_scale = 16.f, int dirs = 0);
int convf1_packed_halfs(int passes);
void convf1_pack(const float *w, int passes, f16 *dst);
int launch_convf1(hipStream_t s, const float *flow, const f16 *wpk, const float *bias, f16 *out, int64_t rows, int P, int h8, int w8, int ldo,
                  int o8_off, float o8_scale, int passes);
int launch_flow_head2(hipStream_t s, const f16 *x, const f16 *w, const float *bias, float *flow, int n, int H, int W, int split = 0);
int launch_put_flow(hipStream_t s, const float *flow, f16 *hx, f16 *hx2, int64_t rows, int ld = 384, int o8_off = 0, float o8_scale = 16.f,
                    int flow_off = 382);
int launch_flow_resize_back(hipStream_t s, const float *in, int N, int ih, int iw, int sh, int sw, float *out, unsigned *maxd);
int launch_upsample(hipStream_t s, const float *flow, const float *mask, int N, int h8, int w8, int pad_l, int pad_t, int sh,
                    int sw, float *out, unsigned *maxd, int factor = 8);
int launch_flow_encode(hipStream_t s, const float *flow, int N, int sh, int sw, const unsigned *maxd, uint8_t *rgb,
                       float *max_out);
int launch_fwdbwd_mask(hipStream_t s, const float *flow, int n, int h, int w, float a1, float a2, uint8_t *mask);
```

prisma_amd/csrc/raft_kernels.hip:

```cpp
#include "raft_kernels.h"

#include <algorithm>

namespace {

inline unsigned nblk(int64_t n, int t = 256) { return (unsigned)((n + t - 1) / t); }

__device__ __forceinline__ float prep_norm(float v, int c, int mode) {
    if (mode == 0) return 2.f * (v / 255.f) - 1.f;
    const float mean = c == 0 ? 0.485f : (c == 1 ? 0.456f : 0.406f), sd = c == 0 ? 0.229f : (c == 1 ? 0.224f : 0.225f);
    return (v / 255.f - mean) / sd;
}

__device__ __forceinline__ void scaled_px(const uint8_t *img, int W, int sy, int sx, int resize, const int *__restrict__ xi,
                                          const int *__restrict__ xc, const int *__restrict__ yi, const int *__restrict__ yc, int (&v)[3]) {
    if (resize) {
        int acc[3] = {0, 0, 0};
#pragma unroll
        for (int ty = 0; ty < 4; ++ty) {
            const uint8_t *row = img + (int64_t)yi[sy * 4 + ty] * W * 3;
            int r[3] = {0, 0, 0};
#pragma unroll
            for (int tx = 0; tx < 4; ++tx) {
                const int o = xi[sx * 4 + tx] * 3, c = xc[sx * 4 + tx];
                r[0] += row[o] * c; r[1] += row[o + 1] * c; r[2] += row[o + 2] * c;
            }
            const int cy = yc[sy * 4 + ty];
            acc[0] += r[0] * cy; acc[1] += r[1] * cy; acc[2] += r[2] * cy;
        }
#pragma unroll
        for (int c = 0; c < 3; ++c) {
            int q = (acc[c] + (1 << 21)) >> 22;
            v[c] = q < 0 ? 0 : (q > 255 ? 255 : q);
        }
    } else {
        const uint8_t *px = img + ((int64_t)sy * W + sx) * 3;
        v[0] = px[0]; v[1] = px[1]; v[2] = px[2];
    }
}

__global__ __launch_bounds__(256) void raft_prep_kernel(const uint8_t *__restrict__ frames, int F, int H, int W, int sh,
                                                        int sw, int Hp, int Wp, int pad_l, int pad_t, int resize,
                                                        const int *__restrict__ xi, const int *__restrict__ xc,
                                                        const int *__restrict__ yi, const int *__restrict__ yc,
                                                        f16 *__restrict__ out, uint8_t *__restrict__ scaled_out, int s2d, int lo_off,
                                                        int lo8_pa, int norm_mode, int isz) {
    const int64_t i = (int64_t)blockIdx.x * blockDim.x + threadIdx.x;
    if (i >= (int64_t)F * Hp * Wp) return;
    const int x = (int)(i % Wp), y = (int)((i / Wp) % Hp), f = (int)(i / ((int64_t)Wp * Hp));
    const uint8_t *img = frames + (int64_t)f * H * W * 3;
    int v[3];
    float vf[3];
    if (isz) {
// ... 181 lines not shown
        lo8_load8((const char *)(a + pix * ldc) + 3 * lo_off + c8 * 8, inv, la);
        if (bsrc) lo8_load8((const char *)(bsrc + pix * ldc) + 3 * lo_off + c8 * 8, inv, lb);
    } else if (lo_off) {
        const f16x8 ta = *(const f16x8 *)(a + o + lo_off);
#pragma unroll
        for (int j = 0; j < 8; ++j) la[j] = (float)ta[j];
        if (bsrc) {
            const f16x8 tb = *(const f16x8 *)(bsrc + o + lo_off);
#pragma unroll
            for (int j = 0; j < 8; ++j) lb[j] = (float)tb[j];
        }
    }
    const f32x4 *st = (const f32x4 *)(sa + ((int64_t)b * C8 * 8 + c8 * 8) * 2);
    f32x4 ms[4], ms2[4];
#pragma unroll
    for (int j = 0; j < 4; ++j) ms[j] = st[j];
    if (bsrc && sb) {
        const f32x4 *s2 = (const f32x4 *)(sb + ((int64_t)b * C8 * 8 + c8 * 8) * 2);
#pragma unroll
        for (int j = 0; j < 4; ++j) ms2[j] = s2[j];
    }
    f16x8 r, rl;
    float rv[8];
#pragma unroll
    for (int j = 0; j < 8; ++j) {
        const float mean = ms[j >> 1][(j & 1) * 2], rstd = ms[j >> 1][(j & 1) * 2 + 1];
        const float xa = lo_off ? (float)va[j] + la[j] : (float)va[j];
        float v = fmaxf((xa - mean) * rstd, 0.f);
        if (bsrc) {
            float w = lo_off ? (float)vb[j] + lb[j] : (float)vb[j];
            if (sb) w = (w - ms2[j >> 1][(j & 1) * 2]) * ms2[j >> 1][(j & 1) * 2 + 1];
            v = fmaxf(v + w, 0.f);
        }
        r[j] = (f16)v;
        rl[j] = (f16)(v - (float)r[j]);
        rv[j] = v;
    }
    *(f16x8 *)(out + o) = r;
    if (lo_off && lo8_pa >= 0) {
        const float shi = __builtin_ldexpf(1.f, lo8_pa), slo = __builtin_ldexpf(1.f, lo8_pa + 12);
        int2 h8, l8;
        h8.x = pb_fp8x4((float)r[0] * shi, (float)r[1] * shi, (float)r[2] * shi, (float)r[3] * shi);
        h8.y = pb_fp8x4((float)r[4] * shi, (float)r[5] * shi, (float)r[6] * shi, (float)r[7] * shi);
        l8.x = pb_fp8x4((rv[0] - (float)r[0]) * slo, (rv[1] - (float)r[1]) * slo, (rv[2] - (float)r[2]) * slo, (rv[3] - (float)r[3]) * slo);
        l8.y = pb_fp8x4((rv[4] - (float)r[4]) * slo, (rv[5] - (float)r[5]) * slo, (rv[6] - (float)r[6]) * slo, (rv[7] - (float)r[7]) * slo);
        char *pb = (char *)(out + pix * ldc);
        *(int2 *)(pb + 2 * lo_off + c8 * 8) = h8;
        *(int2 *)(pb + 3 * lo_off + c8 * 8) = l8;
    } else if (lo_off) *(f16x8 *)(out + o + lo_off) = rl;
}

__global__ __launch_bounds__(256) void init_state_kernel(const f16 *__restrict__ c, float *__restrict__ h32,
                                                          f16 *__restrict__ hx, f16 *__restrict__ hx2, float *__restrict__ flow, int64_t rows,
                                                          int ld, int o8_off, float o8_scale, int inp_off) {
    const int64_t i = (int64_t)blockIdx.x * blockDim.x + threadIdx.x;
    if (i >= rows * 32) return;
    const int c8 = (int)(i % 32);
    const int64_t r = i / 32;
    const f16x8 v = *(const f16x8 *)(c + r * 256 + c8 * 8);
    f16x8 o;
    if (c8 < 16) {
#pragma unroll
        for (int j = 0; j < 8; ++j) {
            const float t = tanhf((float)v[j]);
            h32[r * 128 + c8 * 8 + j] = t;
            o[j] = (f16)t;
        }
    } else {
#pragma unroll
        for (int j = 0; j < 8; ++j) o[j] = (f16)fmaxf((float)v[j], 0.f);
    }
    const int dc = c8 < 16 ? c8 * 8 : inp_off + (c8 - 16) * 8;
    *(f16x8 *)(hx + r * ld + dc) = o;
    if (c8 >= 16) *(f16x8 *)(hx2 + r * ld + dc) = o;
    if (o8_off) {
        int2 o8;
        o8.x = pb_fp8x4((float)o[0] * o8_scale, (float)o[1] * o8_scale, (float)o[2] * o8_scale, (float)o[3] * o8_scale);
        o8.y = pb_fp8x4((float)o[4] * o8_scale, (float)o[5] * o8_scale, (float)o[6] * o8_scale, (float)o[7] * o8_scale);
        *(int2 *)((char *)(hx + r * ld) + o8_off + dc) = o8;
        if (c8 >= 16) *(int2 *)((char *)(hx2 + r * ld) + o8_off + dc) = o8;
    }
    if (c8 == 0) { flow[r * 2] = 0.f; flow[r * 2 + 1] = 0.f; }
}


__global__ __launch_bounds__(256) void avgpool2_nhwc_kernel(const f16 *__restrict__ x, f16 *__restrict__ y, int n, int H, int W, int OH,
                                                            int OW, int C8) {
    const int64_t i = (int64_t)blockIdx.x * blockDim.x + threadIdx.x;
    if (i >= (int64_t)n * OH * OW * C8) return;
    const int c = (int)(i % C8);
    const int64_t pix = i / C8;
    const int ox = (int)(pix % OW), oy = (int)((pix / OW) % OH), b = (int)(pix / ((int64_t)OW * OH));
    const f16 *base = x + (((int64_t)b * H + 2 * oy) * W + 2 * ox) * C8 * 8 + c * 8;
    const f16x8 v00 = *(const f16x8 *)base, v01 = *(const f16x8 *)(base + C8 * 8);
    const f16x8 v10 = *(const f16x8 *)(base + (int64_t)W * C8 * 8), v11 = *(const f16x8 *)(base + (int64_t)(W + 1) * C8 * 8);
    f16x8 o;
#pragma unroll
    for (int j = 0; j < 8; ++j) o[j] = (f16)(0.25f * (((float)v00[j] + (float)v01[j]) + ((float)v10[j] + (float)v11[j])));
    *(f16x8 *)(y + i * 8) = o;
}

__global__ __launch_bounds__(256) void corr_tile_kernel(const f16 *__restrict__ x, f16 *__restrict__ y, int F, int h, int w, int wp,
                                                         int npad) {
    const int64_t i = (int64_t)blockIdx.x * blockDim.x + threadIdx.x;
    if (i >= (int64_t)F * h * w * 32) return;
    const int c = (int)(i & 31);
    const int64_t pix = i >> 5;
    const int px = (int)(pix % w), py = (int)((pix / w) % h), f = (int)(pix / ((int64_t)w * h));
    const f16x8 v = *(const f16x8 *)(x + pix * 256 + c * 8);
    f16x8 o;
#pragma unroll
    for (int j = 0; j < 8; ++j) o[j] = (f16)((float)v[j] * 0.0625f);
    const int row = ((py >> 3) * (wp >> 3) + (px >> 3)) * 64 + (py & 7) * 8 + (px & 7);
    *(f16x8 *)(y + ((int64_t)f * npad + row) * 256 + c * 8) = o;
}

struct PyrPtrs { const f16 *lv[4]; int h[4], w[4], wp[4], ld[4], hp8[4]; };
__device__ __forceinline__ unsigned sel4u(unsigned a0, unsigned a1, unsigned a2, unsigned a3, int l) {
    const unsigned m1 = 0u - (unsigned)(l & 1), m2 = 0u - (unsigned)((l >> 1) & 1);
    const unsigned lo = (a0 & ~m1) | (a1 & m1), hi = (a2 & ~m1) | (a3 & m1);
    return (lo & ~m2) | (hi & m2);
}
__device__ __forceinline__ int sel4(const int (&a)[4], int l) { return (int)sel4u((unsigned)a[0], (unsigned)a[1], (unsigned)a[2], (unsigned)a[3], l); }
__device__ __forceinline__ const f16 *sel4(const f16 *const (&a)[4], int l) {
    const unsigned long long p0 = (unsigned long long)a[0], p1 = (unsigned long long)a[1], p2 = (unsigned long long)a[2], p3 = (unsigned long long)a[3];
    const unsigned lo = sel4u((unsigned)p0, (unsigned)p1, (unsigned)p2, (unsigned)p3, l);
    const unsigned hi = sel4u((unsigned)(p0 >> 32), (unsigned)(p1 >> 32), (unsigned)(p2 >> 32), (unsigned)(p3 >> 32), l);
    return (const f16 *)(((unsigned long long)hi << 32) | lo);
}

__global__ __launch_bounds__(256) void corr_lookup_kernel(PyrPtrs py, const float *__restrict__ flow, int P, int w8,
                                                           f16 *__restrict__ out, int64_t rows, int ldo, int o8_off, float o8_scale) {
    __shared__ __attribute__((aligned(16))) f16 win[28 * 11 * 24];
    __shared__ __attribute__((aligned(8))) f16 tile[7 * 324];
    __shared__ int ci[28 * 18];
    __shared__ float ca[28 * 18];
    const int t = threadIdx.x;
    const int64_t r0 = (int64_t)blockIdx.x * 7;
    {
        f32x2 fl[2];
#pragma unroll
        for (int u = 0; u < 2; ++u) {
            const int idx = t + 256 * u, idc = idx < 28 * 18 ? idx : 0;
            const int pr = (idc / 18) >> 2;
            const int64_t r = r0 + pr < rows ? r0 + pr : rows - 1;
            fl[u] = *(const f32x2 *)(flow + r * 2);
        }
#pragma unroll
        for (int u = 0; u < 2; ++u) {
            const int idx = t + 256 * u, idc = idx < 28 * 18 ? idx : 0;
            const int k = idc % 18, pl = idc / 18, l = pl & 3, pr = pl >> 2;
            const int64_t r = r0 + pr < rows ? r0 + pr : rows - 1;
            const int p = (int)((unsigned)r % (unsigned)P);
            const float inv = 1.f / (float)(1 << l);
            const bool isx = k < 9;
            const float c = (float)(isx ? p % w8 : p / w8) + (isx ? fl[u][0] : fl[u][1]);
            const int dim = isx ? sel4(py.w, l) : sel4(py.h, l);
            const float v = ((2.f * (c * inv + (float)(isx ? k - 4 : k - 13)) / (float)(dim - 1) - 1.f) + 1.f) * 0.5f * (float)(dim - 1);
            const float f = floorf(v);
            if (idx < 28 * 18) {
                ci[idx] = (int)fminf(fmaxf(f, -65536.f), 65536.f);
                ca[idx] = v - f;
            }
        }
    }
    __syncthreads();
    {
        f16x8 wv[4];
        int wdst[4];
#pragma unroll
        for (int u = 0; u < 4; ++u) {
            const int idx = t + 256 * u;
            const int idc = idx < 28 * 33 ? idx : 0;
            const int seg = idc % 3, row = (idc / 3) % 11, pl = idc / 33, l = pl & 3, pr = pl >> 2;
            const int64_t r = r0 + pr < rows ? r0 + pr : rows - 1;
            const int hp8 = sel4(py.hp8, l), wt = sel4(py.wp, l) >> 3;
            const int y = ci[pl * 18 + 9] + row, tx = (ci[pl * 18] >> 3) + seg;
            const bool need = seg < 2 || ci[pl * 18 + 8] + 1 - (ci[pl * 18] & ~7) >= 16;
            const bool ok = idx < 28 * 33 && need && (unsigned)y < (unsigned)hp8 && (unsigned)tx < (unsigned)wt;
            const f16 *src = sel4(py.lv, l) + (ok ? r * (int64_t)sel4(py.ld, l) + ((y >> 3) * wt + tx) * 64 + (y & 7) * 8 : 0);
            const f16x8 ld = *(const __attribute__((address_space(1))) f16x8 *)(unsigned long long)src;
            const f16x8 z = {(f16)0.f, (f16)0.f, (f16)0.f, (f16)0.f, (f16)0.f, (f16)0.f, (f16)0.f, (f16)0.f};
            wv[u] = ok ? ld : z;
            wdst[u] = idx < 28 * 33 ? (pl * 11 + row) * 24 + seg * 8 : -1;
        }
#pragma unroll
        for (int u = 0; u < 4; ++u)
            if (wdst[u] >= 0) *(f16x8 *)(win + wdst[u]) = wv[u];
    }
    __syncthreads();
    if (t < 252) {
        const int li = t % 36, pr = t / 36;
        const int l = li / 9, wi = li - l * 9;
        const int pl = pr * 4 + l, cb = pl * 18;
        const int xb = ci[cb] & ~7, yb = ci[cb + 9];
        int xo = ci[cb + wi] - xb;
        const float ax = ca[cb + wi];
        xo = xo < 0 ? 0 : (xo > 22 ? 22 : xo);
        const f16 *wp = win + pl * 11 * 24 + xo;
        f16 *dst = tile + pr * 324 + l * 81 + wi * 9;
#pragma unroll
        for (int j = 0; j < 9; ++j) {
            int yo = ci[cb + 9 + j] - yb;
            const float ay = ca[cb + 9 + j];
            yo = yo < 0 ? 0 : (yo > 9 ? 9 : yo);
            const float v00 = (float)wp[yo * 24], v01 = (float)wp[yo * 24 + 1];
            const float v10 = (float)wp[yo * 24 + 24], v11 = (float)wp[yo * 24 + 25];
            dst[j] = (f16)(v00 * (1.f - ax) * (1.f - ay) + v01 * ax * (1.f - ay) + v10 * (1.f - ax) * ay + v11 * ax * ay);
        }
    }
    __syncthreads();
    for (int v = t; v < 7 * 81; v += 256) {
        const int pr = v / 81, c4 = v - pr * 81;
        const int64_t r = r0 + pr;
        if (r < rows) {
            const f16x4 o = *(const f16x4 *)(tile + pr * 324 + c4 * 4);
            *(f16x4 *)(out + r * ldo + c4 * 4) = o;
            if (o8_off)
                *(int *)((char *)(out + r * ldo) + o8_off + c4 * 4) = pb_fp8x4((float)o[0] * o8_scale, (float)o[1] * o8_scale, (float)o[2] * o8_scale, (float)o[3] * o8_scale);
        }
    }
}

__global__ void put_flow_kernel(const float *__restrict__ flow, f16 *__restrict__ hx, f16 *__restrict__ hx2, int64_t rows, int ld, int o8_off,
                                float o8_scale, int flow_off) {
    const int64_t r = (int64_t)blockIdx.x * blockDim.x + threadIdx.x;
    if (r >= rows) return;
    f16x2 o;
    o[0] = (f16)flow[r * 2]; o[1] = (f16)flow[r * 2 + 1];
    *(f16x2 *)(hx + r * ld + flow_off) = o;
    *(f16x2 *)(hx2 + r * ld + flow_off) = o;
    if (o8_off) {
        const unsigned short o8 = pb_fp8x2((float)o[0] * o8_scale, (float)o[1] * o8_scale);
        *(unsigned short *)((char *)(hx + r * ld) + o8_off + flow_off) = o8;
        *(unsigned short *)((char *)(hx2 + r * ld) + o8_off + flow_off) = o8;
    }
}


template <bool SPLIT>
__global__ __launch_bounds__(256) void flow_head2_kernel(const f16 *__restrict__ x, const f16 *__restrict__ w, const float *__restrict__ bias,
                                                          float *__restrict__ flow, int nseg, int H, int W, int segw) {
    const int lane = threadIdx.x & 63, half = lane >> 5, cl = lane & 31;
    constexpr int WS = SPLIT ? 512 : 256;
    f16x8 wv[2][9], wl[SPLIT ? 2 : 1][SPLIT ? 9 : 1];
#pragma unroll
    for (int o = 0; o < 2; ++o)
#pragma unroll
        for (int t = 0; t < 9; ++t) {
            wv[o][t] = *(const f16x8 *)(w + (o * 9 + t) * WS + cl * 8);
            if constexpr (SPLIT) wl[o][t] = *(const f16x8 *)(w + (o * 9 + t) * WS + 256 + cl * 8);
        }
    const float b0 = bias[0], b1 = bias[1];
    const int wid = (int)(((int64_t)blockIdx.x * blockDim.x + threadIdx.x) >> 6);
    const int seg = wid * 2 + half;
    if (seg >= nseg) return;
    const int spr = (W + segw - 1) / segw;
    const int sx = seg % spr, y = (seg / spr) % H, img = seg / (spr * H);
    const int xa = sx * segw, xb = xa + segw < W ? xa + segw : W;
    const f16 *base = x + ((int64_t)img * H * W) * 256 + cl * 8;
    f16x8 zero;
#pragma unroll
    for (int j = 0; j < 8; ++j) zero[j] = (f16)0.f;
    auto col = [&](int ix, f16x8 (&c)[3]) {
#pragma unroll
        for (int ky = 0; ky < 3; ++ky) {
            const int iy = y + ky - 1;
            c[ky] = ((unsigned)iy < (unsigned)H && (unsigned)ix < (unsigned)W) ? *(const f16x8 *)(base + ((int64_t)iy * W + ix) * 256) : zero;
// ... 127 lines not shown
        const float h6 = ex_fmul(a, 6.0f);
        const float offs[3] = {0.f, 4.f, 2.f};
        uint8_t o[3];
#pragma unroll
        for (int c = 0; c < 3; ++c) {
            double v = (double)(c == 0 ? h6 : ex_fadd(h6, offs[c]));
            v = fmod(v, 6.0);
            if (v < 0.0) v = ex_dadd(v, 6.0);
            v = ex_dsub(fabs(ex_dsub(v, 3.0)), 1.0);
            v = fmin(fmax(v, 0.0), 1.0);
            v = ex_dadd(ex_dmul(v, (double)rad), (double)ex_fsub(1.0f, rad));
            v = ex_dmul(v, 255.0);
            o[c] = (v == v) ? (uint8_t)(int)v : (uint8_t)0;
        }
        uint8_t *d = rgb + ((int64_t)n * per + i) * 3;
        d[0] = o[0]; d[1] = o[1]; d[2] = o[2];
    }
}

__global__ void fill_u32_kernel(unsigned *p, unsigned v, int n) {
    const int i = blockIdx.x * blockDim.x + threadIdx.x;
    if (i < n) p[i] = v;
}

}

#define LAUNCH_CHECK() do { PB_HIP(hipGetLastError()); return 0; } while (0)

int launch_raft_prep(hipStream_t s, const uint8_t *frames, int F, int H, int W, int sh, int sw, int Hp, int Wp, int pad_l,
                     int pad_t, int resize, const int *xi, const int *xc, const int *yi, const int *yc, f16 *out,
                     uint8_t *scaled_out, int s2d, int lo_off, int lo8_pa, int norm_mode, int isz) {
    hipLaunchKernelGGL(raft_prep_kernel, dim3(nblk((int64_t)F * Hp * Wp)), dim3(256), 0, s, frames, F, H, W, sh, sw, Hp, Wp,
                       pad_l, pad_t, resize, xi, xc, yi, yc, out, scaled_out, s2d, lo_off, lo8_pa, norm_mode, isz);
    LAUNCH_CHECK();
}
int launch_im2col7_flow(hipStream_t s, const float *x, int B, int H, int W, f16 *out, int Kp, int ld, int o8) {
    hipLaunchKernelGGL((im2col7_kernel<float, 2>), dim3(nblk((int64_t)B * H * W * 49)), dim3(256), 0, s, x, B, H, W, 2, 1, H, W,
                       out, Kp, ld ? ld : Kp, o8);
    LAUNCH_CHECK();
}
int in_stats_chunks(int HW) { return (HW + 2047) / 2048; }
int launch_in_stats(hipStream_t s, const f16 *x, int B, int HW, int C, int ldc, float *part, float *stats, int lo_off, int lo8_pa) {
    PB_CHECK(C % 8 == 0 && C <= 256 && 256 % (C / 8) == 0, -1, "instance norm: C=%d unsupported", C);
    const int chunk = 2048, nchunk = in_stats_chunks(HW);
    hipLaunchKernelGGL(in_stats_kernel, dim3(nchunk, B), dim3(256), 0, s, x, HW, C / 8, ldc, part, chunk, lo_off, lo8_pa, stats);
    hipLaunchKernelGGL(in_finalize_kernel, dim3((B * C + 255) / 256), dim3(256), 0, s, part, nchunk, B * C, 1.f / (float)HW, stats);
    LAUNCH_CHECK();
}
int launch_in_apply(hipStream_t s, const f16 *a, const float *sa, const f16 *b, const float *sb, f16 *out, int B, int HW,
                    int C, int ldc, int lo_off, int lo8_pa) {
    hipLaunchKernelGGL(in_apply_kernel, dim3(nblk((int64_t)B * HW * (C / 8))), dim3(256), 0, s, a, sa, b, sb, out, B, HW, C / 8, ldc, lo_off, lo8_pa);
    LAUNCH_CHECK();
}
int launch_init_state(hipStream_t s, const f16 *c, float *h32, f16 *hx, f16 *hx2, float *flow, int64_t rows, int ld, int o8_off, float o8_scale, int inp_off) {
    hipLaunchKernelGGL(init_state_kernel, dim3(nblk(rows * 32)), dim3(256), 0, s, c, h32, hx, hx2, flow, rows, ld, o8_off, o8_scale, inp_off);
    LAUNCH_CHECK();
}
int launch_avgpool2_nhwc(hipStream_t s, const f16 *x, f16 *y, int n, int H, int W, int C) {
    const int OH = H / 2, OW = W / 2;
    hipLaunchKernelGGL(avgpool2_nhwc_kernel, dim3(nblk((int64_t)n * OH * OW * (C / 8))), dim3(256), 0, s, x, y, n, H, W, OH, OW, C / 8);
    LAUNCH_CHECK();
}
int launch_corr_tile(hipStream_t s, const f16 *x, f16 *y, int F, int h, int w, int wp, int npad) {
    hipLaunchKernelGGL(corr_tile_kernel, dim3(nblk((int64_t)F * h * w * 32)), dim3(256), 0, s, x, y, F, h, w, wp, npad);
    LAUNCH_CHECK();
}
void corr_pyramid_geometry(int h8, int w8, CorrGeo &g) {
    g.h[0] = h8; g.w[0] = w8;
    for (int l = 1; l < 4; ++l) { g.h[l] = g.h[l - 1] / 2; g.w[l] = g.w[l - 1] / 2; }
    for (int l = 0; l < 4; ++l) {
        g.wp[l] = (int)round_up(g.w[l], 8);
        g.hp[l] = (int)round_up(g.h[l], 8);
        g.ld[l] = g.hp[l] * g.wp[l];
        if (round_up(g.ld[l], 256) * 50 <= (int64_t)g.ld[l] * 51) g.ld[l] = (int)round_up(g.ld[l], 256);
    }
}
int launch_corr_lookup(hipStream_t s, const f16 *const lv[4], const int h[4], const int w[4], const int wp[4], const int hp[4], const int ld[4],
                       const float *flow, int P, int w8, f16 *out, int64_t rows, int ldo, int o8_off, float o8_scale) {
    PyrPtrs py;
    for (int i = 0; i < 4; ++i) { py.lv[i] = lv[i]; py.h[i] = h[i]; py.w[i] = w[i]; py.wp[i] = wp[i]; py.ld[i] = ld[i]; py.hp8[i] = hp[i]; }
    PB_CHECK(rows < (1LL << 31), -1, "corr_lookup: %lld rows", (long long)rows);
    hipLaunchKernelGGL(corr_lookup_kernel, dim3((unsigned)((rows + 6) / 7)), dim3(256), 0, s, py, flow, P, w8, out, rows, ldo, o8_off, o8_scale);
    LAUNCH_CHECK();
}
constexpr int F1_LD = 120;
__global__ __launch_bounds__(256, 2) void convf1_kernel(const float *__restrict__ flow, const f16 *__restrict__ wpk, const float *__restrict__ bias,
                                                         f16 *__restrict__ out, int64_t rows, int P, int h8, int w8, int ldo, int o8_off, float o8_scale,
                                                         int passes) {
    extern __shared__ __attribute__((aligned(16))) char smem[];
    const int tid = threadIdx.x, lane = tid & 63, li = lane & 31, lh = lane >> 5;
    const int nw16 = passes * 128 * F1_LD / 8;
    for (int i = tid; i < nw16; i += 256) ((f16x8 *)smem)[i] = ((const f16x8 *)wpk)[i];
    __syncthreads();
    float b2[2][2];
#pragma unroll
    for (int g = 0; g < 2; ++g) { b2[g][0] = bias[g * 64 + 2 * li]; b2[g][1] = bias[g * 64 + 2 * li + 1]; }
    const int64_t ntiles = (rows + 31) / 32;
    for (int64_t tile = (int64_t)blockIdx.x * 4 + (tid >> 6); tile < ntiles; tile += (int64_t)gridDim.x * 4) {
        const int64_t m = tile * 32 + li;
        const int64_t mc = m < rows ? m : rows - 1;
        const int64_t n = mc / P;
        const int rem = (int)(mc - n * P), y = rem / w8, x = rem - y * w8;
        const float *fb = flow + n * P * 2;
        f16x8 a[7];
#pragma unroll
        for (int ks = 0; ks < 7; ++ks) {
            f32x2 v[4];
#pragma unroll
            for (int e = 0; e < 4; ++e) {
                const int t = 8 * ks + 4 * lh + e;
                const int ky = (t * 37) >> 8, kx = t - 7 * ky;
                const int iy = y + ky - 3, ix = x + kx - 3;
                const bool ok = t < 49 && (unsigned)iy < (unsigned)h8 && (unsigned)ix < (unsigned)w8;
                const f32x2 z = {0.f, 0.f};
                v[e] = ok ? *(const f32x2 *)(fb + ((int64_t)iy * w8 + ix) * 2) : z;
            }
#pragma unroll
            for (int e = 0; e < 4; ++e) { a[ks][2 * e] = (f16)v[e][0]; a[ks][2 * e + 1] = (f16)v[e][1]; }
        }
        f32x16 acc[4];
#pragma unroll
        for (int j = 0; j < 4; ++j)
#pragma unroll
            for (int r = 0; r < 16; ++r) acc[j][r] = 0.f;
        for (int ps = 0; ps < passes; ++ps) {
            const char *wb = smem + ps * 128 * F1_LD * 2 + li * (F1_LD * 2) + lh * 16;
#pragma unroll
            for (int ks = 0; ks < 7; ++ks)
#pragma unroll
                for (int j = 0; j < 4; ++j) {
                    const f16x8 b = *(const f16x8 *)(wb + j * 32 * (F1_LD * 2) + ks * 32);
                    acc[j] = __builtin_amdgcn_mfma_f32_32x32x16_f16(a[ks], b, acc[j], 0, 0, 0);
                }
        }
#pragma unroll
// ... 149 lines not shown
```

prisma_amd/csrc/volume.hip:

```cpp
#include "common.h"
#include "launch_env.h"
#include "raft_kernels.h"
#include "../../include/prisma_bands.h"

#define LAUNCH_CHECK() do { PB_HIP(hipGetLastError()); return 0; } while (0)

namespace {

#define VOL_BAR()                               \
    do {                                        \
        __builtin_amdgcn_sched_barrier(0);      \
        asm volatile("s_barrier" ::: "memory"); \
        __builtin_amdgcn_sched_barrier(0);      \
    } while (0)

constexpr int VBM = 128, VBN = 64, VNT = 256, VSTAGES = 4, VSTAGE_BYTES = 2 * VBN * 128;

template <int ABL>
__global__ __launch_bounds__(VNT, 2) void corr_volume_kernel(const f16 *__restrict__ A, int M, const f16 *__restrict__ W, int N, int w_rows,
                                                             f16 *__restrict__ out, int64_t ldo, int tiles_per_wg) {
    extern __shared__ __attribute__((aligned(16))) char smem[];
    const int tid = threadIdx.x;
    const int wave = __builtin_amdgcn_readfirstlane(tid >> 6);
    const int lane = tid & 63, li = lane & 31, lh = lane >> 5;

    const int tilesM = (M + VBM - 1) / VBM, tilesN = (N + VBN - 1) / VBN;
    const int nwg = gridDim.x, bid = blockIdx.x;
    const int qd = nwg >> 3, rm = nwg & 7, xcd = bid & 7;
    const int swz = (xcd < rm ? xcd * (qd + 1) : rm * (qd + 1) + (xcd - rm) * qd) + (bid >> 3);
    const int grp = swz / tilesM, tile_m = swz - grp * tilesM;
    const int m0 = tile_m * VBM + wave * 32;
    const int nt0 = grp * tiles_per_wg;
    const int ntl = (tilesN - nt0) < tiles_per_wg ? (tilesN - nt0) : tiles_per_wg;
    if (ntl <= 0) return;

    f16x8 af[16];
    {
        const int row = m0 + li;
        const f16 *src = A + (int64_t)(row < M ? row : M - 1) * 256 + lh * 8;
#pragma unroll
        for (int ks = 0; ks < 16; ++ks) af[ks] = *(const f16x8 *)(src + ks * 16);
    }

    const __amdgpu_buffer_rsrc_t rsW = make_rsrc(W, (unsigned)((int64_t)w_rows * 512));
    const int srow = tid >> 3, cg = (tid & 7) ^ ((tid >> 4) & 7);
    int b_voff[2];
#pragma unroll
    for (int i = 0; i < 2; ++i) {
        const int r = srow + i * 32;
        b_voff[i] = (2 * (r & 31) + (r >> 5)) * 512 + cg * 16;
    }
    auto stage = [&](int g) {
        if (ABL & 4) return;
        const int nt = nt0 + (g >> 1), h = g & 1;
        char *dst = smem + (g & (VSTAGES - 1)) * VSTAGE_BYTES + wave * 1024;
        const int soff = nt * (VBN * 512) + h * 256;
#pragma unroll
        for (int kk = 0; kk < 2; ++kk)
#pragma unroll
            for (int i = 0; i < 2; ++i) glds16_buf(rsW, b_voff[i], soff + kk * 128, dst + kk * (VBN * 128) + i * 4096);
    };

    const int fsw = (li >> 1) & 7;
    const int b_off[2] = {li * 128, (32 + li) * 128};

    f32x16 acc[2];
#pragma unroll
    for (int j = 0; j < 2; ++j)
#pragma unroll
        for (int r = 0; r < 16; ++r) acc[j][r] = 0.f;

    const int G = ntl * 2;
    asm volatile("s_waitcnt vmcnt(0)" ::: "memory");
    stage(0);
    stage(1);
    if (G > 2) stage(2);
    f16x8 qa[8], qb[8];
#define PB_VOL_C(KK, KS) ((KK) * (VBN * 128) + ((2 * (KS) + lh) ^ fsw) * 16)
#define PB_VOL_RD(Q, SB, KK, KS)                                                  \
    Q[2 * (KS)] = *(const f16x8 *)((SB) + b_off[0] + PB_VOL_C(KK, KS));           \
    Q[2 * (KS) + 1] = *(const f16x8 *)((SB) + b_off[1] + PB_VOL_C(KK, KS));
#define PB_VOL_MM(Q, A0, KS)                                                                       \
    acc[0] = __builtin_amdgcn_mfma_f32_32x32x16_f16(af[(A0) + (KS)], Q[2 * (KS)], acc[0], 0, 0, 0);     \
    acc[1] = __builtin_amdgcn_mfma_f32_32x32x16_f16(af[(A0) + (KS)], Q[2 * (KS) + 1], acc[1], 0, 0, 0);
#define PB_VOL_PIN() __builtin_amdgcn_sched_barrier(0)
    f16x2 pk[16];
    int pk_n = -1;
    const int rows_w = (M - m0) < 32 ? (M - m0 < 0 ? 0 : M - m0) : 32;
    const int ldb = (int)ldo * 2;
    const uint64_t ob = (uint64_t)(out + (int64_t)m0 * ldo);
    const uint64_t ob_u = ((uint64_t)(unsigned)__builtin_amdgcn_readfirstlane((int)(ob >> 32)) << 32) | (unsigned)__builtin_amdgcn_readfirstlane((int)ob);
    const __amdgpu_buffer_rsrc_t rsO = make_rsrc((const void *)ob_u, (unsigned)__builtin_amdgcn_readfirstlane(rows_w * ldb));
    const int vo_lane = 4 * lh * ldb + 4 * li;
    constexpr int VO_NONE = 0x7ffff000;
    int vo_st = VO_NONE;
    const bool rows_full = __builtin_amdgcn_readfirstlane(rows_w) == 32;
    auto flush = [&]() {
        if (ABL & 1) return;
        if (rows_full) {
#pragma unroll
            for (int r = 0; r < 16; ++r)
                __builtin_amdgcn_raw_buffer_store_b32(__builtin_bit_cast(unsigned, pk[r]), rsO, vo_st, ((r & 3) + 8 * (r >> 2)) * ldb, 0);
        } else {
#pragma unroll
            for (int r = 0; r < 16; ++r) {
                const int row = (r & 3) + 8 * (r >> 2);
                __builtin_amdgcn_raw_buffer_store_b32(__builtin_bit_cast(unsigned, pk[r]), rsO, row + 4 * lh < rows_w ? vo_st : VO_NONE, row * ldb, 0);
            }
        }
    };
    unsigned keep = 0;
    for (int j = 0; j < ntl; ++j) {
        const int g = 2 * j;
        if (g + 2 < G) asm volatile("s_waitcnt vmcnt(4)" ::: "memory");
        else asm volatile("s_waitcnt vmcnt(0)" ::: "memory");
        VOL_BAR();
        if (g + 3 < G) stage(g + 3);
        flush();
        const char *sb0 = smem + (g & (VSTAGES - 1)) * VSTAGE_BYTES, *sb1 = smem + ((g + 1) & (VSTAGES - 1)) * VSTAGE_BYTES;
        if (!(ABL & 2)) {
#pragma unroll
            for (int ks = 0; ks < 4; ++ks) { PB_VOL_RD(qa, sb0, 0, ks) }
#pragma unroll
            for (int ks = 0; ks < 4; ++ks) { PB_VOL_RD(qb, sb0, 1, ks) }
            PB_VOL_PIN();
#pragma unroll
            for (int ks = 0; ks < 4; ++ks) { PB_VOL_MM(qa, 0, ks) PB_VOL_RD(qa, sb1, 0, ks) PB_VOL_PIN(); }
#pragma unroll
            for (int ks = 0; ks < 4; ++ks) { PB_VOL_MM(qb, 4, ks) PB_VOL_RD(qb, sb1, 1, ks) PB_VOL_PIN(); }
        }
        VOL_BAR();
        if (g + 4 < G) stage(g + 4);
        if (!(ABL & 2)) {
#pragma unroll
            for (int ks = 0; ks < 4; ++ks) { PB_VOL_MM(qa, 8, ks) }
#pragma unroll
            for (int ks = 0; ks < 4; ++ks) { PB_VOL_MM(qb, 12, ks) }
        }
        pk_n = (nt0 + j) * VBN + 2 * li;
        vo_st = pk_n < N ? vo_lane + (nt0 + j) * (VBN * 2) : VO_NONE;
#pragma unroll
        for (int r = 0; r < 16; ++r) {
            pk[r] = f16x2{(f16)acc[0][r], (f16)acc[1][r]};
            acc[0][r] = 0.f; acc[1][r] = 0.f;
            if (ABL & 1) keep ^= __builtin_bit_cast(unsigned, pk[r]);
        }
    }
#undef PB_VOL_C
#undef PB_VOL_RD
#undef PB_VOL_MM
#undef PB_VOL_PIN
    flush();
    if ((ABL & 1) && keep == 0x12345679u) out[0] = (f16)1.f;
}

}

int launch_corr_volume(hipStream_t s, const f16 *A, int M, const f16 *W, int N, int w_rows, f16 *out, int64_t ldo) {
    PB_CHECK(A && W && out && M > 0 && N > 0 && N % 8 == 0 && ldo >= N && w_rows >= N && ldo < (1 << 24), PB_ERR_ARG, "corr_volume: bad arguments");
    const int smem = VSTAGES * VSTAGE_BYTES;
#ifdef PB_DIAG
    const int abl = launch_env().vol_abl;
#else
    const int abl = 0;
#endif
    const int tilesM = (M + VBM - 1) / VBM, tilesN = (N + VBN - 1) / VBN;
    int groups = (2048 + tilesM - 1) / tilesM;
    groups = groups < 1 ? 1 : (groups > tilesN ? tilesN : groups);
    const int tpw = (tilesN + groups - 1) / groups;
    groups = (tilesN + tpw - 1) / tpw;
#define PB_VOL_LAUNCH(X)                                                                                                  \
    {                                                                                                                     \
        static PbLdsLimit lds;                                                                                            \
        if (int rc = pb_lds_limit(lds, (const void *)corr_volume_kernel<X>, smem)) return rc;                             \
        hipLaunchKernelGGL(corr_volume_kernel<X>, dim3(tilesM * groups), dim3(VNT), smem, s, A, M, W, N, w_rows, out, ldo, tpw); \
    }
    switch (abl) {
#ifdef PB_DIAG
        case 1: PB_VOL_LAUNCH(1); break;
        case 2: PB_VOL_LAUNCH(2); break;
        case 4: PB_VOL_LAUNCH(4); break;
        case 5: PB_VOL_LAUNCH(5); break;
        case 6: PB_VOL_LAUNCH(6); break;
#endif
        default: PB_VOL_LAUNCH(0);
    }
#undef PB_VOL_LAUNCH
    LAUNCH_CHECK();
}
```

prisma_amd/engine.py:

```python
from __future__ import annotations

import ctypes as C
from typing import Dict, List, Optional, Tuple

import numpy as np

from . import _lib
from ._lib import check
from .synth import DEPTH_CFGS, MASK_CFGS, DepthCfg, MaskCfg


def _ptr(a: Optional[np.ndarray]):
    return None if a is None else a.ctypes.data_as(C.c_void_p)


def _f32(a) -> np.ndarray:
    return np.ascontiguousarray(a, dtype=np.float32)


VERTEX_DTYPE = np.dtype([("x", "<f4"), ("y", "<f4"), ("z", "<f4"), ("red", "u1"), ("green", "u1"), ("blue", "u1")])


def device_count() -> int:
    return _lib.load().pb_device_count()
# ... 266 lines not shown
    def rgb_shape(self, h: int, w: int) -> tuple:
        return (i420_bytes(h, w),) if self.rgb_format == "i420" else (h, w, 3)

    def _flow_rgb_shape(self, H: int, W: int, sh: int, sw: int) -> tuple:
        return self.rgb_shape(H, W) if self.rgb_full else self.rgb_shape(sh, sw)

    def set_option(self, key: str, value: int):
        check(self.lib.pb_set_option(self.ctx, key.encode(), int(value)))


    def set_profiling(self, timing: bool = True, debug_stages: bool = False, accumulate: bool = False):
        check(self.lib.pb_set_profiling(self.ctx, (1 if timing else 0) | (2 if debug_stages else 0) | (4 if accumulate else 0)))

    _stage_sym: Optional[str] = None
    _stage_cap = 1 << 26
    _stage_squeeze = True

    def stage(self, name: str, cap: Optional[int] = None) -> np.ndarray:
        cap = self._stage_cap if cap is None else cap
        out = np.empty(cap, np.float32)
        shape = (C.c_int64 * 4)()
        n = check(getattr(self.lib, self._stage_sym)(self.ctx, name.encode(), _ptr(out), cap, shape))
        dims = [int(s) for s in shape]
        while self._stage_squeeze and len(dims) > 1 and dims[-1] == 1:
            dims.pop()
        return out[:n].reshape(dims).copy()

    def kernel_stats(self) -> List[dict]:
        arr = (_lib.pb_kernel_stat * 64)()
        n = check(self.lib.pb_get_kernel_stats(self.ctx, arr, 64))
        return [dict(name=arr[i].name.decode(), ms=arr[i].ms, flops=arr[i].flops, exec_flops=arr[i].exec_flops, bytes=arr[i].bytes,
                     launches=arr[i].launches) for i in range(n)]


_SPLIT_INFO = ("pw", "pa", "mx3", "mx2", "sa", "sw", "tapin", "K", "cw", "Cseg", "ldo", "lo8", "lo8_pa")


def _split_info(info, M: int) -> dict:
    d = dict(zip(_SPLIT_INFO, list(info)))
    d["M"] = M
    return d


def _epi_info(info) -> dict:
    return dict(zip(("pw", "pa", "mx2", "sw", "K", "nk16", "mx3", "splitk"), list(info)))


def raft_geometry(h8: int, w8: int) -> List[dict]:
    geo = (C.c_int * 20)()
    check(_lib.load().pb_op_raft_geometry(h8, w8, geo))
    return [dict(h=geo[l * 5], w=geo[l * 5 + 1], wp=geo[l * 5 + 2], hp=geo[l * 5 + 3], ld=geo[l * 5 + 4]) for l in range(4)]


def gm_geometry(h8: int, w8: int, splits: int = 2) -> dict:
    P, wh, ww = h8 * w8, h8 // splits, w8 // splits
    return dict(h8=h8, w8=w8, P=P, wh=wh, ww=ww, Lw=wh * ww, ldv=-(-(wh * ww) // 32) * 32, ldvP=-(-P // 32) * 32, ns=splits)


def gm_tables(h8: int, w8: int):
    pos = np.empty((h8 * w8, 128), np.float32)
    reg = np.empty((4, (h8 // 2) * (w8 // 2)), np.int8)
    check(_lib.load().pb_op_gm_tables(h8, w8, _ptr(pos), _ptr(reg)))
    return pos, reg


def gm_tables_n(h: int, w: int, splits: int):
    pos = np.empty((h * w, 128), np.float32)
    reg = np.empty((splits * splits, (h // splits) * (w // splits)), np.int8)
    check(_lib.load().pb_op_gm_tables_n(h, w, splits, _ptr(pos), _ptr(reg)))
    return pos, reg


class Ops(_Ctx):

    def __init__(self, device: int = 0):
        super().__init__()
        check(self.lib.pb_create(C.byref(self.ctx), device, b"ops", None, 0, None, 0))

    def gemm(self, A, W, bias=None, act: int = 0, tile: int = 0) -> np.ndarray:
        A, W = _f32(A), _f32(W)
        M, K = A.shape
        N = W.shape[0]
        out = np.empty((M, N), np.float32)
        b = None if bias is None else _f32(bias)
        check(self.lib.pb_op_gemm(self.ctx, _ptr(A), _ptr(W), _ptr(b), _ptr(out), M, N, K, act, tile))
        return out

    def corr_volume(self, A, W, ldo: int = 0, guard_rows: int = 32) -> np.ndarray:
        A, W = _f32(A), _f32(W)
        M, N = A.shape[0], W.shape[0]
        ldo = ldo or N
        out = np.empty((M + guard_rows, ldo), np.float32)
        check(self.lib.pb_op_corr_volume(self.ctx, _ptr(A), M, _ptr(W), N, ldo, guard_rows, _ptr(out)))
        return out

    def gemm_bench(self, M: int, N: int, K: int, tile: int = 0, epi: int = 0, iters: int = 20) -> float:
        ms = C.c_double()
        check(self.lib.pb_op_gemm_bench(self.ctx, M, N, K, tile, epi, iters, C.byref(ms)))
        return ms.value

    def attention_bench(self, B: int, heads: int, N: int, variant: int = 0, iters: int = 10) -> float:
        ms = C.c_double()
        check(self.lib.pb_op_attention_bench(self.ctx, B, heads, N, variant, iters, C.byref(ms)))
        return ms.value

    def layernorm(self, x, g, b) -> np.ndarray:
        x, g, b = _f32(x), _f32(g), _f32(b)
        out = np.empty_like(x)
        check(self.lib.pb_op_layernorm(self.ctx, _ptr(x), _ptr(g), _ptr(b), _ptr(out), x.shape[0], x.shape[1]))
        return out

    def attention128(self, q, k, v, region=None) -> np.ndarray:
        q, k, v = _f32(q), _f32(k), _f32(v)
        B, L, D = q.shape
        assert D == 128 and k.shape == q.shape and v.shape == q.shape
        out = np.empty_like(q)
        rg = None if region is None else np.ascontiguousarray(region, np.int8)
        check(self.lib.pb_op_attention128(self.ctx, _ptr(q), _ptr(k), _ptr(v), _ptr(rg), _ptr(out), B, L))
        return out

    def attention128_split(self, q, k, v, region=None, kxor: int = 0) -> np.ndarray:
        q, k, v = _f32(q), _f32(k), _f32(v)
        B, L, D = q.shape
        vc = v.shape[2]
        assert D == 128 and k.shape == q.shape and v.shape[:2] == (B, L) and vc in (32, 128)
        out = np.empty((B, L, vc), np.float32)
        rg = None if region is None else np.ascontiguousarray(region, np.int8)
        check(self.lib.pb_op_attention128_split(self.ctx, _ptr(q), _ptr(k), _ptr(v), _ptr(rg), 0 if rg is None else rg.shape[0], _ptr(out),
                                                B, L, vc, kxor))
        return out

    def attention(self, q, k, v) -> np.ndarray:
        q, k, v = _f32(q), _f32(k), _f32(v)
        B, Hh, N, d = q.shape
        assert d == 64
        out = np.empty_like(q)
        check(self.lib.pb_op_attention(self.ctx, _ptr(q), _ptr(k), _ptr(v), _ptr(out), B, Hh, N))
        return out

    def conv2d(self, x, w, bias=None, stride=1, pad=None, relu_in=False, relu_out=False) -> np.ndarray:
        x, w = _f32(x), _f32(w)
        B, Ci, H, W = x.shape
        Co, _, ks, _ = w.shape
        pad = ks // 2 if pad is None else pad
        OH, OW = (H + 2 * pad - ks) // stride + 1, (W + 2 * pad - ks) // stride + 1
        out = np.empty((B, Co, OH, OW), np.float32)
# ... 921 lines not shown
```

Measured before the change: 129.1.

## Store RAFT correlation pyramid in 8x64 blocked tiles and add blocked lookup kernel

Adds a blocked layout for the correlation volume. Each group of 8 source pixels is stored as contiguous 8x64 tiles, the volume kernel writes in this order, and a new lookup kernel reads one 8-pixel block per workgroup. The aim is better locality and coalescing in the per-iteration correlation lookup, which samples windows at neighbouring pixels. It is on by default when the volume kernel path is active. It also folds the per-pair init_state launches into one launch, and adds test entry points for the blocked layout.

```diff
diff --git a/include/prisma_bands.h b/include/prisma_bands.h
--- a/include/prisma_bands.h
+++ b/include/prisma_bands.h
@@ -178,6 +178,8 @@
                int M, int N, int K, int act , int tile );
 int pb_op_gemm_bench(pb_ctx *ctx, int M, int N, int K, int tile, int epi, int iters, double *ms_out);
 int pb_op_corr_volume(pb_ctx *ctx, const float *A, int M, const float *W, int N, int ldo, int guard_rows, float *out);
+int pb_op_corr_volume_blocked(pb_ctx *ctx, const float *A, int M, const float *W, int N, int ldo, int guard_halfs, void *out);
+int pb_op_corr_layout_index(int layout, int P, int pld, int64_t *out);
 int pb_op_attention_bench(pb_ctx *ctx, int B, int heads, int N, int variant, int iters, double *ms_out);
 int pb_op_layernorm(pb_ctx *ctx, const float *x, const float *g, const float *b, float *y, int rows, int D);
 int pb_op_attention(pb_ctx *ctx, const float *q, const float *k, const float *v, float *o,
diff --git a/prisma_amd/_lib.py b/prisma_amd/_lib.py
--- a/prisma_amd/_lib.py
+++ b/prisma_amd/_lib.py
@@ -115,6 +115,8 @@
     "pb_op_gemm": (C.c_int, [_P, _P, _P, _P, _P, C.c_int, C.c_int, C.c_int, C.c_int, C.c_int]),
     "pb_op_gemm_bench": (C.c_int, [_P, C.c_int, C.c_int, C.c_int, C.c_int, C.c_int, C.c_int, C.POINTER(C.c_double)]),
     "pb_op_corr_volume": (C.c_int, [_P, _P, C.c_int, _P, C.c_int, C.c_int, C.c_int, _P]),
+    "pb_op_corr_volume_blocked": (C.c_int, [_P, _P, C.c_int, _P, C.c_int, C.c_int, C.c_int, _P]),
+    "pb_op_corr_layout_index": (C.c_int, [C.c_int, C.c_int, C.c_int, _P]),
     "pb_op_attention_bench": (C.c_int, [_P, C.c_int, C.c_int, C.c_int, C.c_int, C.c_int, C.POINTER(C.c_double)]),
     "pb_op_layernorm": (C.c_int, [_P, _P, _P, _P, _P, C.c_int, C.c_int]),
     "pb_op_attention": (C.c_int, [_P, _P, _P, _P, _P, C.c_int, C.c_int, C.c_int]),
diff --git a/prisma_amd/csrc/abi.hip b/prisma_amd/csrc/abi.hip
--- a/prisma_amd/csrc/abi.hip
+++ b/prisma_amd/csrc/abi.hip
@@ -670,6 +670,12 @@
         PB_CHECK(c->pending.empty(), PB_ERR_STATE, "option '%s': a submission of this ctx is still outstanding (pb_wait first)", key);
         (key[0] == 'f' ? c->frames_i420 : key[8] == 'i' ? c->rgb_out_i420 : c->rgb_out_full) = value;
     }
+    else if (!strcmp(key, "corr_layout")) {
+        PB_CHECK(value == 0 || value == 1, PB_ERR_ARG, "option '%s' is 0 or 1, not %d", key, value);
+        PB_CHECK(c->pending.empty(), PB_ERR_STATE, "option '%s': a submission of this ctx is still outstanding (pb_wait first)", key);
+        c->corr_layout = value;
+        if (RaftEngine *e = dynamic_cast<RaftEngine *>(c->flow)) e->set_corr_layout(value);
+    }
     else if (!strcmp(key, "tile_n96")) pb_gemm_set_n96(value);
     else PB_CHECK(false, PB_ERR_ARG, "unknown option '%s'", key);
     return 0;
diff --git a/prisma_amd/csrc/abi_ctx.h b/prisma_amd/csrc/abi_ctx.h
--- a/prisma_amd/csrc/abi_ctx.h
+++ b/prisma_amd/csrc/abi_ctx.h
@@ -124,6 +124,7 @@
     int gemm_tile = TILE_AUTO, conv_tile = TILE_AUTO;
     int op_splitk = 0;
     int host_chunk = 0;
+    int corr_layout = 1;
     ChunkPipe pipe;
     MaskPipe mpipe;
     std::deque<hipEvent_t> pending;
diff --git a/prisma_amd/csrc/abi_ops.hip b/prisma_amd/csrc/abi_ops.hip
--- a/prisma_amd/csrc/abi_ops.hip
+++ b/prisma_amd/csrc/abi_ops.hip
@@ -4,6 +4,7 @@
 #include <vector>
 
 #include "abi_ctx.h"
+#include "corr_layout.h"
 #include "gmflow_engine.h"
 #include "mask_kernels.h"
 #include "zoe_kernels.h"
@@ -156,12 +157,13 @@
         return 0;
     }
 
-    int lookup(const float *fmap1, const float *fmap2, const float *flow, int n, int h8, int w8, int o8, int guard_rows, void *out, float *levels) {
+    int lookup(const float *fmap1, const float *fmap2, const float *flow, int n, int h8, int w8, int o8, int guard_rows, void *out, float *levels,
+               int layout) {
         PB_CHECK(h8 >= 16 && w8 >= 16, PB_ERR_ARG, "op_raft_lookup: a %d x %d grid is too small (the 4-level pyramid needs >= 16 x 16)", h8, w8);
         CorrGeo g;
         corr_pyramid_geometry(h8, w8, g);
         const int P = h8 * w8;
-        const int64_t rows = (int64_t)n * P;
+        const int64_t rows = (int64_t)n * P, Pv = corr_layout_rows(layout, P);
         const size_t slack = 1 << 20;
         const int ldo = o8 ? 576 : 384;
         DevMem f1, f2, dflow, dout, fpool[4], ftile[4], pyr[4];
@@ -171,7 +173,7 @@
         PB_TRY(preset(dout, (size_t)(rows + guard_rows) * ldo * 2));
         const f16 *lv[4];
         for (int l = 0; l < 4; ++l) {
-            PB_TRY(pyr[l].alloc((size_t)rows * g.ld[l] * 2 + slack));
+            PB_TRY(pyr[l].alloc((size_t)n * Pv * g.ld[l] * 2 + slack));
             if (l) PB_TRY(fpool[l].alloc((size_t)round_up((int64_t)n * g.h[l] * g.w[l], 256) * 256 * 2 + slack));
             PB_TRY(ftile[l].alloc((size_t)(n * (int64_t)g.ld[l] + 256) * 256 * 2 + slack));
             lv[l] = pyr[l].as<f16>();
@@ -183,20 +185,23 @@
         for (int i = 0; i < n; ++i)
             for (int l = 0; l < 4; ++l)
                 PB_TRY(launch_corr_volume(stream, f1.as<f16>() + (int64_t)i * P * 256, P, ftile[l].as<f16>() + (int64_t)i * g.ld[l] * 256, g.ld[l], g.ld[l],
-                                          pyr[l].as<f16>() + (int64_t)i * P * g.ld[l], g.ld[l]));
+                                          pyr[l].as<f16>() + (int64_t)i * Pv * g.ld[l], g.ld[l], layout));
         PB_TRY(launch_corr_lookup(stream, lv, g.h, g.w, g.wp, g.hp, g.ld, dflow.as<float>(), P, w8, dout.as<f16>(), rows, ldo, o8 ? 768 : 0,
-                                  (float)(1 << kMx2Pa)));
+                                  (float)(1 << kMx2Pa), layout));
         PB_TRY(finish(out, dout, (size_t)(rows + guard_rows) * ldo * 2));
         if (levels) {
             float *dst = levels;
             for (int l = 0; l < 4; ++l) {
-                std::vector<f16> h((size_t)rows * g.ld[l]);
+                std::vector<f16> h((size_t)n * Pv * g.ld[l]);
                 PB_HIP(hipMemcpy(h.data(), pyr[l].p, h.size() * 2, hipMemcpyDeviceToHost));
                 const int wt = g.wp[l] >> 3;
-                for (int64_t r = 0; r < rows; ++r)
+                for (int64_t r = 0; r < rows; ++r) {
+                    const f16 *hn = h.data() + (size_t)(r / P) * Pv * g.ld[l];
+                    const int p = (int)(r % P);
                     for (int y = 0; y < g.h[l]; ++y)
                         for (int x = 0; x < g.w[l]; ++x)
-                            *dst++ = (float)h[(size_t)r * g.ld[l] + ((y >> 3) * wt + (x >> 3)) * 64 + (y & 7) * 8 + (x & 7)];
+                            *dst++ = (float)hn[corr_layout_index(layout, p, ((y >> 3) * wt + (x >> 3)) * 64 + (y & 7) * 8 + (x & 7), g.ld[l])];
+                }
             }
         }
         return 0;
@@ -1271,6 +1276,33 @@
     return 0;
 }
 
+int pb_op_corr_volume_blocked(pb_ctx *c, const float *A, int M, const float *W, int N, int ldo, int guard_halfs, void *out) {
+    PB_CHECK(c && A && W && out && M > 0 && N > 0 && N % 8 == 0 && ldo >= N && ldo % 64 == 0 && guard_halfs >= 0, PB_ERR_ARG, "op_corr_volume_blocked: bad arguments");
+    PB_HIP(hipSetDevice(c->device));
+    const int64_t Np = round_up(N, 64);
+    const size_t halfs = (size_t)corr_layout_rows(CORR_BLOCKED, M) * ldo + guard_halfs;
+    DevMem a32, w32, a16, w16, o16;
+    PB_TRY(a32.alloc((size_t)M * 256 * 4)); PB_TRY(w32.alloc((size_t)N * 256 * 4));
+    PB_TRY(a16.alloc((size_t)M * 256 * 2)); PB_TRY(w16.alloc((size_t)Np * 256 * 2));
+    PB_TRY(o16.alloc(halfs * 2));
+    PB_HIP(hipMemcpy(a32.p, A, (size_t)M * 256 * 4, hipMemcpyHostToDevice));
+    PB_HIP(hipMemcpy(w32.p, W, (size_t)N * 256 * 4, hipMemcpyHostToDevice));
+    PB_HIP(hipMemsetAsync(w16.p, 0, (size_t)Np * 256 * 2, c->stream));
+    PB_HIP(hipMemsetAsync(o16.p, 0x7e, halfs * 2, c->stream));
+    PB_TRY(launch_f32_to_f16(c->stream, a32.as<float>(), a16.as<f16>(), M, 256, 256));
+    PB_TRY(launch_f32_to_f16(c->stream, w32.as<float>(), w16.as<f16>(), N, 256, 256));
+    PB_TRY(launch_corr_volume(c->stream, a16.as<f16>(), M, w16.as<f16>(), N, (int)Np, o16.as<f16>(), ldo, CORR_BLOCKED));
+    PB_HIP(hipStreamSynchronize(c->stream));
+    PB_HIP(hipMemcpy(out, o16.p, halfs * 2, hipMemcpyDeviceToHost));
+    return 0;
+}
+int pb_op_corr_layout_index(int layout, int P, int pld, int64_t *out) {
+    PB_CHECK(out && P > 0 && pld > 0 && pld % 64 == 0 && (layout == CORR_ROWMAJOR || layout == CORR_BLOCKED), PB_ERR_ARG, "op_corr_layout_index: bad arguments");
+    for (int p = 0; p < P; ++p)
+        for (int cc = 0; cc < pld; ++cc) out[(size_t)p * pld + cc] = corr_layout_index(layout, p, cc, pld);
+    return 0;
+}
+
 int pb_op_gemm_bench(pb_ctx *c, int M, int N, int K, int tile, int epi, int iters, double *ms_out) {
     PB_CHECK(c && M > 0 && N > 0 && K > 0 && K % 64 == 0 && N % 8 == 0 && iters > 0 && ms_out, PB_ERR_ARG, "gemm_bench: bad arguments");
     PB_HIP(hipSetDevice(c->device));
@@ -1633,7 +1665,7 @@
                       float *levels) {
     PB_CHECK(c && fmap1 && fmap2 && flow && out && n > 0 && guard_rows >= 0, PB_ERR_ARG, "op_raft_lookup: bad arguments");
     RAFT_OP_ENGINE(e);
-    return e.lookup(fmap1, fmap2, flow, n, h8, w8, o8, guard_rows, out, levels);
+    return e.lookup(fmap1, fmap2, flow, n, h8, w8, o8, guard_rows, out, levels, launch_env().volume ? c->corr_layout : CORR_ROWMAJOR);
 }
 int pb_op_raft_lookup_otf(pb_ctx *c, const float *fmap1, const float *fmap2, const float *flow, int n, int h8, int w8, int o8, int guard_rows, void *out) {
     PB_CHECK(c && fmap1 && fmap2 && flow && out && n > 0 && guard_rows >= 0, PB_ERR_ARG, "op_raft_lookup_otf: bad arguments");
diff --git a/prisma_amd/csrc/corr_layout.h b/prisma_amd/csrc/corr_layout.h
--- /dev/null
+++ b/prisma_amd/csrc/corr_layout.h
@@ -0,0 +1,17 @@
+#pragma once
+#if defined(__HIPCC__)
+#define PB_CL __device__ __host__ __forceinline__
+#else
+#define PB_CL inline
+#endif
+
+enum { CORR_ROWMAJOR = 0, CORR_BLOCKED = 1 };
+
+PB_CL long long corr_layout_rows(int layout, int P) { return layout == CORR_BLOCKED ? ((long long)P + 7) / 8 * 8 : P; }
+
+PB_CL long long corr_blocked_tile(int pblk, int j, int T) { return ((long long)pblk * T + j) * 512; }
+
+PB_CL long long corr_layout_index(int layout, int p, int c, int pld) {
+    if (layout != CORR_BLOCKED) return (long long)p * pld + c;
+    return corr_blocked_tile(p >> 3, c >> 6, pld >> 6) + (p & 7) * 64 + (c & 63);
+}
diff --git a/prisma_amd/csrc/raft_engine.h b/prisma_amd/csrc/raft_engine.h
--- a/prisma_amd/csrc/raft_engine.h
+++ b/prisma_amd/csrc/raft_engine.h
@@ -8,6 +8,7 @@
     int infer(const uint8_t *frames, int F, int H, int W, float scale, int iters, int backward, float *flow_out, uint8_t *rgb_out,
               float *maxdisp, uint8_t *mask_out = nullptr, float alpha1 = 0.05f, float alpha2 = 0.5f) override;
     void set_alternate_corr(int on) { alt_corr_ = on ? 1 : 0; }
+    void set_corr_layout(int blocked) { corr_layout_ = blocked ? 1 : 0; }
     int chunk_pairs(int wanted, int H, int W, float scale, int dirs) const override;
 
   private:
@@ -22,6 +23,9 @@
     f16 *gz_[2] = {}, *gq_[2] = {};
 
     int alt_corr_ = 0;
+    int corr_layout_ = 1;
+    int vol_layout() const;
+    int plan_word() const { return alt_corr_ | (vol_layout() << 1); }
     int lh_[4] = {0, 0, 0, 0}, lw_[4] = {0, 0, 0, 0};
     f16 *fmap_ = nullptr, *ctx_ = nullptr;
     f16 *pyr_[4] = {};
diff --git a/prisma_amd/csrc/raft_engine.hip b/prisma_amd/csrc/raft_engine.hip
--- a/prisma_amd/csrc/raft_engine.hip
+++ b/prisma_amd/csrc/raft_engine.hip
@@ -1,5 +1,6 @@
 #include "raft_engine.h"
 #include "flow_chunk.h"
+#include "corr_layout.h"
 
 #include <math.h>
 #include <string.h>
@@ -121,8 +122,10 @@
     return 0;
 }
 
+int RaftEngine::vol_layout() const { return corr_layout_ && !alt_corr_ && launch_env().volume ? CORR_BLOCKED : CORR_ROWMAJOR; }
+
 int RaftEngine::prepare(int F, int H, int W, float scale, int dirs) {
-    if (plan_.covers(F, H, W, scale, dirs, alt_corr_)) return 0;
+    if (plan_.covers(F, H, W, scale, dirs, plan_word())) return 0;
     PB_HIP(hipStreamSynchronize(stream));
     plan_.clear();
     geometry(H, W, scale, 8);
@@ -139,7 +142,7 @@
         fmap_ = (f16 *)carve((size_t)round_up((int64_t)F * P_, 256) * 256 * 2 + slack);
         ctx_ = (f16 *)carve((size_t)round_up((int64_t)F * P_, 256) * 256 * 2);
         for (int l = 0; l < 4; ++l) {
-            pyr_[l] = alt_corr_ ? nullptr : (f16 *)carve((size_t)ND * P_ * pld_[l] * 2 + slack);
+            pyr_[l] = alt_corr_ ? nullptr : (f16 *)carve((size_t)ND * corr_layout_rows(vol_layout(), P_) * pld_[l] * 2 + slack);
             fpool_[l] = l == 0 ? nullptr : (f16 *)carve((size_t)round_up((int64_t)F * lh_[l] * lw_[l], 256) * 256 * 2 + slack);
             ftile_[l] = alt_corr_ ? nullptr : (f16 *)carve((size_t)(F * (int64_t)pld_[l] + 256) * 256 * 2 + slack);
         }
@@ -163,7 +166,7 @@
         return 0;
     });
     if (r || (r = upload_resize_tables(H, W, scale))) return r;
-    plan_.set(F, H, W, scale, dirs, alt_corr_);
+    plan_.set(F, H, W, scale, dirs, plan_word());
     return 0;
 }
 
@@ -202,28 +205,26 @@
         });
         if (r) return r;
     }
-    for (int i = 0; i < F - 1; ++i)
+    const int layout = vol_layout();
+    for (int i = 0; i < F - 1 && !alt_corr_; ++i)
         for (int d = 0; d < dirs; ++d) {
             const int n = i * dirs + d;
-            for (int l = 0; l < 4 && !alt_corr_; ++l) {
+            for (int l = 0; l < 4; ++l) {
                 GemmArgs a;
                 a.A = fmap_ + (int64_t)(i + d) * P_ * 256; a.lda = 256; a.M = P_;
                 a.W = ftile_[l] + (int64_t)(i + 1 - d) * pld_[l] * 256;
                 a.K = 256; a.N = pld_[l];
-                a.out = pyr_[l] + (int64_t)n * P_ * pld_[l]; a.ldo = pld_[l]; a.zero = zero_;
+                a.out = pyr_[l] + (int64_t)n * corr_layout_rows(layout, P_) * pld_[l]; a.ldo = pld_[l]; a.zero = zero_;
                 const double flops = 2.0 * P_ * (double)lh_[l] * lw_[l] * 256, bytes = 2.0 * ((double)P_ * 256 + (double)pld_[l] * 256 + (double)P_ * pld_[l]);
                 if (!launch_env().volume)
                     r = timed_gemm(F_GEMM, flops, bytes, [&] { return launch_gemm(stream, A_DENSE, EPI_STD, TILE_AUTO, a); });
                 else
-                    r = timed(F_GEMM, flops, bytes, [&] { return launch_corr_volume(stream, a.A, a.M, a.W, a.N, a.N, a.out, a.ldo); }, "corr_volume_kernel");
+                    r = timed(F_GEMM, flops, bytes, [&] { return launch_corr_volume(stream, a.A, a.M, a.W, a.N, a.N, a.out, a.ldo, layout); }, "corr_volume_kernel");
                 if (r) return r;
             }
-            r = timed(F_ELT, 0, 0, [&] {
-                return launch_init_state(stream, ctx_ + (int64_t)(i + d) * P_ * 256, h32_ + (int64_t)n * P_ * 128, hx_ + (int64_t)n * P_ * Lhx,
-                                         hx2_ + (int64_t)n * P_ * Lhx, flow_ + (int64_t)n * P_ * 2, P_, Lhx, upd8_ ? 768 : 0, s8, hoist_ ? 256 : 128);
-            });
-            if (r) return r;
-        }
+        }
+    r = timed(F_ELT, 0, 0, [&] { return launch_init_state(stream, ctx_, h32_, hx_, hx2_, flow_, rows, Lhx, upd8_ ? 768 : 0, s8, hoist_ ? 256 : 128, P_, dirs); });
+    if (r) return r;
 
     if (debug && (r = snapshot("net0", h32_, (size_t)ND * P_ * 128 * 4, Stage::f32_rows(nullptr, ND, P_, 128)))) return r;
 
@@ -248,7 +249,7 @@
                 return launch_corr_lookup_otf(stream, fmap_, tg, lh_, lw_, flow_, P_, w8_, corr_, rows, Lhx, upd8_ ? 768 : 0, s8, dirs);
             }, "corr_lookup_otf_kernel");
         } else {
-            r = timed(F_ELT, 0, 0, [&] { return launch_corr_lookup(stream, pyr_, lh_, lw_, lwp_, lhp_, pld_, flow_, P_, w8_, corr_, rows, Lhx, upd8_ ? 768 : 0, s8); });
+            r = timed(F_ELT, 0, 0, [&] { return launch_corr_lookup(stream, pyr_, lh_, lw_, lwp_, lhp_, pld_, flow_, P_, w8_, corr_, rows, Lhx, upd8_ ? 768 : 0, s8, layout); });
         }
         if (r) return r;
         if (debug && it == 0 && (r = snapshot("corr0", corr_, (size_t)ND * P_ * Lhx * 2, Stage::f16_nhwc(nullptr, ND, 324, h8_, w8_, Lhx)))) return r;
diff --git a/prisma_amd/csrc/raft_kernels.h b/prisma_amd/csrc/raft_kernels.h
--- a/prisma_amd/csrc/raft_kernels.h
+++ b/prisma_amd/csrc/raft_kernels.h
@@ -11,14 +11,16 @@
 int launch_in_apply(hipStream_t s, const f16 *a, const float *sa, const f16 *b, const float *sb, f16 *out, int B, int HW,
                     int C, int ldc, int lo_off = 0, int lo8_pa = -1);
 int launch_init_state(hipStream_t s, const f16 *c, float *h32, f16 *hx, f16 *hx2, float *flow, int64_t rows, int ld = 384, int o8_off = 0,
-                      float o8_scale = 16.f, int inp_off = 128);
+                      float o8_scale = 16.f, int inp_off = 128,
+                      int P = 0, int dirs = 0);
 int launch_avgpool2_nhwc(hipStream_t s, const f16 *x, f16 *y, int n, int H, int W, int C);
 int launch_corr_tile(hipStream_t s, const f16 *x, f16 *y, int F, int h, int w, int wp, int npad);
-int launch_corr_volume(hipStream_t s, const f16 *A, int M, const f16 *W, int N, int w_rows, f16 *out, int64_t ldo);
+int launch_corr_volume(hipStream_t s, const f16 *A, int M, const f16 *W, int N, int w_rows, f16 *out, int64_t ldo, int layout = 0);
 struct CorrGeo { int h[4], w[4], wp[4], hp[4], ld[4]; };
 void corr_pyramid_geometry(int h8, int w8, CorrGeo &g);
 int launch_corr_lookup(hipStream_t s, const f16 *const lv[4], const int h[4], const int w[4], const int wp[4], const int hp[4], const int ld[4],
-                       const float *flow, int P, int w8, f16 *out, int64_t rows, int ldo = 384, int o8_off = 0, float o8_scale = 16.f);
+                       const float *flow, int P, int w8, f16 *out, int64_t rows, int ldo = 384, int o8_off = 0, float o8_scale = 16.f,
+                       int layout = 0);
 int launch_corr_lookup_otf(hipStream_t s, const f16 *fmap_src, const f16 *const fmap_tgt[4], const int h[4], const int w[4], const float *flow, int P,
                            int w8, f16 *out, int64_t rows, int ldo = 384, int o8_off = 0, float o8_scale = 16.f, int dirs = 0);
 int convf1_packed_halfs(int passes);
diff --git a/prisma_amd/csrc/raft_kernels.hip b/prisma_amd/csrc/raft_kernels.hip
--- a/prisma_amd/csrc/raft_kernels.hip
+++ b/prisma_amd/csrc/raft_kernels.hip
@@ -1,4 +1,5 @@
 #include "raft_kernels.h"
+#include "corr_layout.h"
 
 #include <algorithm>
 
@@ -286,12 +287,17 @@
 
 __global__ __launch_bounds__(256) void init_state_kernel(const f16 *__restrict__ c, float *__restrict__ h32,
                                                           f16 *__restrict__ hx, f16 *__restrict__ hx2, float *__restrict__ flow, int64_t rows,
-                                                          int ld, int o8_off, float o8_scale, int inp_off) {
+                                                          int ld, int o8_off, float o8_scale, int inp_off, int P, int dirs) {
     const int64_t i = (int64_t)blockIdx.x * blockDim.x + threadIdx.x;
     if (i >= rows * 32) return;
     const int c8 = (int)(i % 32);
     const int64_t r = i / 32;
-    const f16x8 v = *(const f16x8 *)(c + r * 256 + c8 * 8);
+    int64_t cr = r;
+    if (dirs) {
+        const int n = (int)(r / P);
+        cr = (int64_t)(n / dirs + n % dirs) * P + (r - (int64_t)n * P);
+    }
+    const f16x8 v = *(const f16x8 *)(c + cr * 256 + c8 * 8);
     f16x8 o;
     if (c8 < 16) {
 #pragma unroll
@@ -363,6 +369,31 @@
     return (const f16 *)(((unsigned long long)hi << 32) | lo);
 }
 
+__device__ __forceinline__ void lookup_sample(int p, int w8, float fx, float fy, int k, int l, int dim, int &ci, float &ca) {
+    const float inv = 1.f / (float)(1 << l);
+    const bool isx = k < 9;
+    const float c = (float)(isx ? p % w8 : p / w8) + (isx ? fx : fy);
+    const float v = ((2.f * (c * inv + (float)(isx ? k - 4 : k - 13)) / (float)(dim - 1) - 1.f) + 1.f) * 0.5f * (float)(dim - 1);
+    const float f = floorf(v);
+    ci = (int)fminf(fmaxf(f, -65536.f), 65536.f);
+    ca = v - f;
+}
+__device__ __forceinline__ f16 lookup_blend(const f16 *wp, int yo, float ax, float ay, bool last) {
+    const float v00 = (float)wp[yo * 24], v01 = (float)wp[yo * 24 + 1];
+    const float v10 = (float)wp[yo * 24 + 24], v11 = (float)wp[yo * 24 + 25];
+    float s = __builtin_fmaf(v00 * (1.f - ax), 1.f - ay, (v01 * ax) * (1.f - ay));
+    s = __builtin_fmaf(v10 * (1.f - ax), ay, s);
+    const float a11 = v11 * ax;
+    if (last) {
+        unsigned o;
+        asm("v_fma_mixlo_f16 %0, %1, %2, %3" : "=v"(o) : "v"(ay), "v"(a11), "v"(s));
+        return __builtin_bit_cast(f16, (unsigned short)o);
+    }
+    float r = __builtin_fmaf(a11, ay, s);
+    asm("" : "+v"(r));
+    return (f16)r;
+}
+
 __global__ __launch_bounds__(256) void corr_lookup_kernel(PyrPtrs py, const float *__restrict__ flow, int P, int w8,
                                                            f16 *__restrict__ out, int64_t rows, int ldo, int o8_off, float o8_scale) {
     __shared__ __attribute__((aligned(16))) f16 win[28 * 11 * 24];
@@ -386,15 +417,12 @@
             const int k = idc % 18, pl = idc / 18, l = pl & 3, pr = pl >> 2;
             const int64_t r = r0 + pr < rows ? r0 + pr : rows - 1;
             const int p = (int)((unsigned)r % (unsigned)P);
-            const float inv = 1.f / (float)(1 << l);
-            const bool isx = k < 9;
-            const float c = (float)(isx ? p % w8 : p / w8) + (isx ? fl[u][0] : fl[u][1]);
-            const int dim = isx ? sel4(py.w, l) : sel4(py.h, l);
-            const float v = ((2.f * (c * inv + (float)(isx ? k - 4 : k - 13)) / (float)(dim - 1) - 1.f) + 1.f) * 0.5f * (float)(dim - 1);
-            const float f = floorf(v);
+            int cif;
+            float caf;
+            lookup_sample(p, w8, fl[u][0], fl[u][1], k, l, k < 9 ? sel4(py.w, l) : sel4(py.h, l), cif, caf);
             if (idx < 28 * 18) {
-                ci[idx] = (int)fminf(fmaxf(f, -65536.f), 65536.f);
-                ca[idx] = v - f;
+                ci[idx] = cif;
+                ca[idx] = caf;
             }
         }
     }
@@ -438,9 +466,7 @@
             int yo = ci[cb + 9 + j] - yb;
             const float ay = ca[cb + 9 + j];
             yo = yo < 0 ? 0 : (yo > 9 ? 9 : yo);
-            const float v00 = (float)wp[yo * 24], v01 = (float)wp[yo * 24 + 1];
-            const float v10 = (float)wp[yo * 24 + 24], v11 = (float)wp[yo * 24 + 25];
-            dst[j] = (f16)(v00 * (1.f - ax) * (1.f - ay) + v01 * ax * (1.f - ay) + v10 * (1.f - ax) * ay + v11 * ax * ay);
+            dst[j] = lookup_blend(wp, yo, ax, ay, j == 8);
         }
     }
     __syncthreads();
@@ -448,6 +474,102 @@
         const int pr = v / 81, c4 = v - pr * 81;
         const int64_t r = r0 + pr;
         if (r < rows) {
+            const f16x4 o = *(const f16x4 *)(tile + pr * 324 + c4 * 4);
+            *(f16x4 *)(out + r * ldo + c4 * 4) = o;
+            if (o8_off)
+                *(int *)((char *)(out + r * ldo) + o8_off + c4 * 4) = pb_fp8x4((float)o[0] * o8_scale, (float)o[1] * o8_scale, (float)o[2] * o8_scale, (float)o[3] * o8_scale);
+        }
+    }
+}
+
+__global__ __launch_bounds__(256) void corr_lookup_blocked_kernel(PyrPtrs py, const float *__restrict__ flow, int P, int w8, int nb8,
+                                                                   f16 *__restrict__ out, int ldo, int o8_off, float o8_scale) {
+    __shared__ __attribute__((aligned(16))) f16 win[32 * 11 * 24];
+    __shared__ __attribute__((aligned(8))) f16 tile[8 * 324];
+    __shared__ int ci[32 * 18];
+    __shared__ float ca[32 * 18];
+    const int t = threadIdx.x;
+    const int g = blockIdx.x, n = g / nb8, p0 = (g - n * nb8) * 8;
+    const int64_t r0 = (int64_t)n * P + p0;
+    const int nv = P - p0 < 8 ? P - p0 : 8;
+    {
+        f32x2 fl[3];
+#pragma unroll
+        for (int u = 0; u < 3; ++u) {
+            const int idx = t + 256 * u, idc = idx < 32 * 18 ? idx : 0;
+            const int pr = (idc / 18) >> 2;
+            fl[u] = *(const f32x2 *)(flow + (r0 + (pr < nv ? pr : nv - 1)) * 2);
+        }
+#pragma unroll
+        for (int u = 0; u < 3; ++u) {
+            const int idx = t + 256 * u, idc = idx < 32 * 18 ? idx : 0;
+            const int k = idc % 18, pl = idc / 18, l = pl & 3, pr = pl >> 2;
+            int cif;
+            float caf;
+            lookup_sample(p0 + (pr < nv ? pr : nv - 1), w8, fl[u][0], fl[u][1], k, l, k < 9 ? sel4(py.w, l) : sel4(py.h, l), cif, caf);
+            if (idx < 32 * 18) {
+                ci[idx] = cif;
+                ca[idx] = caf;
+            }
+        }
+    }
+    __syncthreads();
+    {
+        const int l = __builtin_amdgcn_readfirstlane(t >> 6), q = (t & 63) >> 3, yy = t & 7;
+        const int pl = q * 4 + l;
+        const int hp8 = sel4(py.hp8, l), wt = sel4(py.wp, l) >> 3;
+        const int x0 = ci[pl * 18], y0 = ci[pl * 18 + 9];
+        const bool third = ci[pl * 18 + 8] + 1 - (x0 & ~7) >= 16;
+        const f16 *lv0 = sel4(py.lv, l), *grp = lv0 + corr_blocked_tile(g, 0, sel4(py.ld, l) >> 6);
+        f16x8 wv[9];
+        int wdst[9];
+#pragma unroll
+        for (int u = 0; u < 9; ++u) {
+            const int tr = u / 3, tc = u % 3;
+            const int wr = tr * 8 + yy - (y0 & 7);
+            const int y = y0 + wr, tx = (x0 >> 3) + tc;
+            const bool slot = (unsigned)wr < 11u;
+            const bool ok = slot && q < nv && (tc < 2 || third) && (unsigned)y < (unsigned)hp8 && (unsigned)tx < (unsigned)wt;
+            const f16 *src = ok ? grp + ((int)corr_blocked_tile(0, (y >> 3) * wt + tx, 0) + q * 64 + yy * 8) : lv0;
+            const f16x8 ld = __builtin_nontemporal_load((const __attribute__((address_space(1))) f16x8 *)(unsigned long long)src);
+            const f16x8 z = {(f16)0.f, (f16)0.f, (f16)0.f, (f16)0.f, (f16)0.f, (f16)0.f, (f16)0.f, (f16)0.f};
+            wv[u] = ok ? ld : z;
+            wdst[u] = slot ? (pl * 11 + wr) * 24 + tc * 8 : -1;
+        }
+#pragma unroll
+        for (int u = 0; u < 9; ++u)
+            if (wdst[u] >= 0) *(f16x8 *)(win + wdst[u]) = wv[u];
+    }
+    __syncthreads();
+#pragma unroll
+    for (int u = 0; u < 4; ++u) {
+        const int v = t + 256 * u;
+        if (v < 3 * 288) {
+            const int jg = v / 288, rem = v - jg * 288;
+            const int li = rem % 36, pr = rem / 36;
+            const int l = li / 9, wi = li - l * 9;
+            const int pl = pr * 4 + l, cb = pl * 18;
+            const int xb = ci[cb] & ~7, yb = ci[cb + 9];
+            int xo = ci[cb + wi] - xb;
+            const float ax = ca[cb + wi];
+            xo = xo < 0 ? 0 : (xo > 22 ? 22 : xo);
+            const f16 *wp = win + pl * 11 * 24 + xo;
+            f16 *dst = tile + pr * 324 + l * 81 + wi * 9;
+#pragma unroll
+            for (int jj = 0; jj < 3; ++jj) {
+                const int j = jg * 3 + jj;
+                int yo = ci[cb + 9 + j] - yb;
+                const float ay = ca[cb + 9 + j];
+                yo = yo < 0 ? 0 : (yo > 9 ? 9 : yo);
+                dst[j] = lookup_blend(wp, yo, ax, ay, j == 8);
+            }
+        }
+    }
+    __syncthreads();
+    for (int v = t; v < 8 * 81; v += 256) {
+        const int pr = v / 81, c4 = v - pr * 81;
+        const int64_t r = r0 + pr;
+        if (pr < nv) {
             const f16x4 o = *(const f16x4 *)(tile + pr * 324 + c4 * 4);
             *(f16x4 *)(out + r * ldo + c4 * 4) = o;
             if (o8_off)
@@ -681,8 +803,10 @@
     hipLaunchKernelGGL(in_apply_kernel, dim3(nblk((int64_t)B * HW * (C / 8))), dim3(256), 0, s, a, sa, b, sb, out, B, HW, C / 8, ldc, lo_off, lo8_pa);
     LAUNCH_CHECK();
 }
-int launch_init_state(hipStream_t s, const f16 *c, float *h32, f16 *hx, f16 *hx2, float *flow, int64_t rows, int ld, int o8_off, float o8_scale, int inp_off) {
-    hipLaunchKernelGGL(init_state_kernel, dim3(nblk(rows * 32)), dim3(256), 0, s, c, h32, hx, hx2, flow, rows, ld, o8_off, o8_scale, inp_off);
+int launch_init_state(hipStream_t s, const f16 *c, float *h32, f16 *hx, f16 *hx2, float *flow, int64_t rows, int ld, int o8_off, float o8_scale, int inp_off,
+                      int P, int dirs) {
+    PB_CHECK(dirs == 0 || (P > 0 && rows % P == 0 && dirs <= 2), -1, "init_state: %lld rows in blocks of %d, %d directions", (long long)rows, P, dirs);
+    hipLaunchKernelGGL(init_state_kernel, dim3(nblk(rows * 32)), dim3(256), 0, s, c, h32, hx, hx2, flow, rows, ld, o8_off, o8_scale, inp_off, P, dirs);
     LAUNCH_CHECK();
 }
 int launch_avgpool2_nhwc(hipStream_t s, const f16 *x, f16 *y, int n, int H, int W, int C) {
@@ -705,11 +829,18 @@
     }
 }
 int launch_corr_lookup(hipStream_t s, const f16 *const lv[4], const int h[4], const int w[4], const int wp[4], const int hp[4], const int ld[4],
-                       const float *flow, int P, int w8, f16 *out, int64_t rows, int ldo, int o8_off, float o8_scale) {
+                       const float *flow, int P, int w8, f16 *out, int64_t rows, int ldo, int o8_off, float o8_scale, int layout) {
     PyrPtrs py;
     for (int i = 0; i < 4; ++i) { py.lv[i] = lv[i]; py.h[i] = h[i]; py.w[i] = w[i]; py.wp[i] = wp[i]; py.ld[i] = ld[i]; py.hp8[i] = hp[i]; }
     PB_CHECK(rows < (1LL << 31), -1, "corr_lookup: %lld rows", (long long)rows);
-    hipLaunchKernelGGL(corr_lookup_kernel, dim3((unsigned)((rows + 6) / 7)), dim3(256), 0, s, py, flow, P, w8, out, rows, ldo, o8_off, o8_scale);
+    if (layout == CORR_BLOCKED) {
+        PB_CHECK(P > 0 && rows % P == 0, -1, "corr_lookup: %lld rows are no whole pair-directions of %d", (long long)rows, P);
+        for (int i = 0; i < 4; ++i) PB_CHECK(ld[i] % 64 == 0 && ld[i] >= hp[i] * wp[i], -1, "corr_lookup: level %d stride %d", i, ld[i]);
+        const int nb8 = (P + 7) / 8;
+        hipLaunchKernelGGL(corr_lookup_blocked_kernel, dim3((unsigned)(rows / P * nb8)), dim3(256), 0, s, py, flow, P, w8, nb8, out, ldo, o8_off, o8_scale);
+    } else {
+        hipLaunchKernelGGL(corr_lookup_kernel, dim3((unsigned)((rows + 6) / 7)), dim3(256), 0, s, py, flow, P, w8, out, rows, ldo, o8_off, o8_scale);
+    }
     LAUNCH_CHECK();
 }
 constexpr int F1_LD = 120;
diff --git a/prisma_amd/csrc/volume.hip b/prisma_amd/csrc/volume.hip
--- a/prisma_amd/csrc/volume.hip
+++ b/prisma_amd/csrc/volume.hip
@@ -1,6 +1,7 @@
 #include "common.h"
 #include "launch_env.h"
 #include "raft_kernels.h"
+#include "corr_layout.h"
 #include "../../include/prisma_bands.h"
 
 #define LAUNCH_CHECK() do { PB_HIP(hipGetLastError()); return 0; } while (0)
@@ -18,7 +19,7 @@
 
 template <int ABL>
 __global__ __launch_bounds__(VNT, 2) void corr_volume_kernel(const f16 *__restrict__ A, int M, const f16 *__restrict__ W, int N, int w_rows,
-                                                             f16 *__restrict__ out, int64_t ldo, int tiles_per_wg) {
+                                                             f16 *__restrict__ out, int64_t ldo, int layout, int tiles_per_wg) {
     extern __shared__ __attribute__((aligned(16))) char smem[];
     const int tid = threadIdx.x;
     const int wave = __builtin_amdgcn_readfirstlane(tid >> 6);
@@ -88,10 +89,12 @@
     int pk_n = -1;
     const int rows_w = (M - m0) < 32 ? (M - m0 < 0 ? 0 : M - m0) : 32;
     const int ldb = (int)ldo * 2;
-    const uint64_t ob = (uint64_t)(out + (int64_t)m0 * ldo);
+    const int rs = layout == CORR_BLOCKED ? 128 : ldb, gs = layout == CORR_BLOCKED ? (int)corr_blocked_tile(1, 0, (int)(ldo >> 6)) * 2 : 8 * ldb;
+    const int ts = layout == CORR_BLOCKED ? 1024 : VBN * 2;
+    const uint64_t ob = (uint64_t)((char *)out + (int64_t)(m0 >> 3) * gs);
     const uint64_t ob_u = ((uint64_t)(unsigned)__builtin_amdgcn_readfirstlane((int)(ob >> 32)) << 32) | (unsigned)__builtin_amdgcn_readfirstlane((int)ob);
-    const __amdgpu_buffer_rsrc_t rsO = make_rsrc((const void *)ob_u, (unsigned)__builtin_amdgcn_readfirstlane(rows_w * ldb));
-    const int vo_lane = 4 * lh * ldb + 4 * li;
+    const __amdgpu_buffer_rsrc_t rsO = make_rsrc((const void *)ob_u, (unsigned)__builtin_amdgcn_readfirstlane(layout == CORR_BLOCKED ? ((rows_w + 7) >> 3) * gs : rows_w * ldb));
+    const int vo_lane = 4 * lh * rs + 4 * li;
     constexpr int VO_NONE = 0x7ffff000;
     int vo_st = VO_NONE;
     const bool rows_full = __builtin_amdgcn_readfirstlane(rows_w) == 32;
@@ -100,12 +103,12 @@
         if (rows_full) {
 #pragma unroll
             for (int r = 0; r < 16; ++r)
-                __builtin_amdgcn_raw_buffer_store_b32(__builtin_bit_cast(unsigned, pk[r]), rsO, vo_st, ((r & 3) + 8 * (r >> 2)) * ldb, 0);
+                __builtin_amdgcn_raw_buffer_store_b32(__builtin_bit_cast(unsigned, pk[r]), rsO, vo_st, (r & 3) * rs + (r >> 2) * gs, 0);
         } else {
 #pragma unroll
             for (int r = 0; r < 16; ++r) {
                 const int row = (r & 3) + 8 * (r >> 2);
-                __builtin_amdgcn_raw_buffer_store_b32(__builtin_bit_cast(unsigned, pk[r]), rsO, row + 4 * lh < rows_w ? vo_st : VO_NONE, row * ldb, 0);
+                __builtin_amdgcn_raw_buffer_store_b32(__builtin_bit_cast(unsigned, pk[r]), rsO, row + 4 * lh < rows_w ? vo_st : VO_NONE, (r & 3) * rs + (r >> 2) * gs, 0);
             }
         }
     };
@@ -138,7 +141,7 @@
             for (int ks = 0; ks < 4; ++ks) { PB_VOL_MM(qb, 12, ks) }
         }
         pk_n = (nt0 + j) * VBN + 2 * li;
-        vo_st = pk_n < N ? vo_lane + (nt0 + j) * (VBN * 2) : VO_NONE;
+        vo_st = pk_n < N ? vo_lane + (nt0 + j) * ts : VO_NONE;
 #pragma unroll
         for (int r = 0; r < 16; ++r) {
             pk[r] = f16x2{(f16)acc[0][r], (f16)acc[1][r]};
@@ -156,8 +159,10 @@
 
 }
 
-int launch_corr_volume(hipStream_t s, const f16 *A, int M, const f16 *W, int N, int w_rows, f16 *out, int64_t ldo) {
+int launch_corr_volume(hipStream_t s, const f16 *A, int M, const f16 *W, int N, int w_rows, f16 *out, int64_t ldo, int layout) {
     PB_CHECK(A && W && out && M > 0 && N > 0 && N % 8 == 0 && ldo >= N && w_rows >= N && ldo < (1 << 24), PB_ERR_ARG, "corr_volume: bad arguments");
+    PB_CHECK(layout == CORR_ROWMAJOR || (layout == CORR_BLOCKED && ldo % 64 == 0), PB_ERR_ARG, "corr_volume: layout %d with a row of %lld entries", layout,
+             (long long)ldo);
     const int smem = VSTAGES * VSTAGE_BYTES;
 #ifdef PB_DIAG
     const int abl = launch_env().vol_abl;
@@ -173,7 +178,7 @@
     {                                                                                                                     \
         static PbLdsLimit lds;                                                                                            \
         if (int rc = pb_lds_limit(lds, (const void *)corr_volume_kernel<X>, smem)) return rc;                             \
-        hipLaunchKernelGGL(corr_volume_kernel<X>, dim3(tilesM * groups), dim3(VNT), smem, s, A, M, W, N, w_rows, out, ldo, tpw); \
+        hipLaunchKernelGGL(corr_volume_kernel<X>, dim3(tilesM * groups), dim3(VNT), smem, s, A, M, W, N, w_rows, out, ldo, layout, tpw); \
     }
     switch (abl) {
 #ifdef PB_DIAG
diff --git a/prisma_amd/engine.py b/prisma_amd/engine.py
--- a/prisma_amd/engine.py
+++ b/prisma_amd/engine.py
@@ -342,6 +342,12 @@
     return [dict(h=geo[l * 5], w=geo[l * 5 + 1], wp=geo[l * 5 + 2], hp=geo[l * 5 + 3], ld=geo[l * 5 + 4]) for l in range(4)]
 
 
+def corr_layout_index(layout: int, P: int, pld: int) -> np.ndarray:
+    out = np.empty((P, pld), np.int64)
+    check(_lib.load().pb_op_corr_layout_index(layout, P, pld, _ptr(out)))
+    return out
+
+
 def gm_geometry(h8: int, w8: int, splits: int = 2) -> dict:
     P, wh, ww = h8 * w8, h8 // splits, w8 // splits
     return dict(h8=h8, w8=w8, P=P, wh=wh, ww=ww, Lw=wh * ww, ldv=-(-(wh * ww) // 32) * 32, ldvP=-(-P // 32) * 32, ns=splits)
@@ -382,6 +388,14 @@
         ldo = ldo or N
         out = np.empty((M + guard_rows, ldo), np.float32)
         check(self.lib.pb_op_corr_volume(self.ctx, _ptr(A), M, _ptr(W), N, ldo, guard_rows, _ptr(out)))
+        return out
+
+    def corr_volume_blocked(self, A, W, ldo: int = 0, guard_halfs: int = 4096) -> np.ndarray:
+        A, W = _f32(A), _f32(W)
+        M, N = A.shape[0], W.shape[0]
+        ldo = ldo or N
+        out = np.empty(-(-M // 8) * 8 * ldo + guard_halfs, np.float16)
+        check(self.lib.pb_op_corr_volume_blocked(self.ctx, _ptr(A), M, _ptr(W), N, ldo, guard_halfs, _ptr(out)))
         return out
 
     def gemm_bench(self, M: int, N: int, K: int, tile: int = 0, epi: int = 0, iters: int = 20) -> float:
```

Measured after the change: 131.6, median of 6. 2.0% higher.
